# illini-robomaster/irmv_detection

Hardware: NVIDIA B200
Metric: frames/s (640^2 YOLOv8n+NMS+PnP) (higher is better)
Workload: dtype f16

## Files before the change

### irmv_detection_b200/csrc/common.cuh

```cuda
#pragma once
#include <cuda_fp16.h>
#include <cuda_runtime.h>
#include <stdint.h>

#include <string>
#include <vector>

namespace irmv {

constexpr int kNet = 640;
constexpr int kInC = 8;
constexpr int kRegMax = 16;
constexpr int kNumAnchors = 8400;
constexpr int kClsPad = 16;
constexpr int kMaxCand = 4096;

__host__ __device__ inline int pr_wp(int W) { return W + 1; }
__host__ __device__ inline long long pr_pixels(int B, int H, int W) { return ((long long)B * (H + 1) + 1) * (W + 1); }
__host__ __device__ inline long long pr_index(int b, int y, int x, int H, int W) {
  return ((long long)b * (H + 1) + 1 + y) * (W + 1) + x;
}
constexpr int kGuardFront = 384;
constexpr int kGuardBack = 1024;

void set_error(const std::string &msg);
bool cuda_ok(cudaError_t e, const char *what, const char *file, int line);

#define IRMV_CUDA(call)                                              \
  do {                                                               \
    if (!::irmv::cuda_ok((call), #call, __FILE__, __LINE__)) return 1; \
  } while (0)

struct PreprocessParams {
  const uint8_t *src;
  const uint8_t *const *src_indirect;
  __half *dst;
  uint8_t *rotated;
  int n, src_w, src_h;
  int frame0;
  int rev_order;
  int chan_order, rotate180, resize_mode, quantize_u8;
  int pad_x, pad_y, new_w, new_h;
};
inline void letterbox_geometry(int src_w, int src_h, int resize_mode, int *pad_x, int *pad_y, int *new_w, int *new_h) {
  *pad_x = *pad_y = 0; *new_w = *new_h = kNet;
  if (resize_mode != 1) return;
  const double rw = (double)kNet / src_w, rh = (double)kNet / src_h, r = rw < rh ? rw : rh;
  *new_w = (int)(src_w * r + 0.5); *new_h = (int)(src_h * r + 0.5);
  if (*new_w > kNet) *new_w = kNet;
  if (*new_h > kNet) *new_h = kNet;
  const double dw = (kNet - *new_w) / 2.0, dh = (kNet - *new_h) / 2.0;
  *pad_x = (int)(dw - 0.1 + 0.5); *pad_y = (int)(dh - 0.1 + 0.5);
  if (*pad_x < 0) *pad_x = 0;
  if (*pad_y < 0) *pad_y = 0;
}
cudaError_t launch_preprocess(const PreprocessParams &p, cudaStream_t s);
cudaError_t launch_rotate(const PreprocessParams &p, cudaStream_t s);
cudaError_t launch_stem(const PreprocessParams &p, const float *w, const float *bias, const uint32_t *fast_tab, __half *out,
                        long long out_pstride, __half *out2, long long out2_pstride, cudaStream_t s);
bool stem_bayer2x_applies(const PreprocessParams &p);
std::vector<uint32_t> stem_bayer2x_tables(const float *w, const float *bias, int src_h, int chan_order, int rotate180);
cudaError_t launch_stem_bayer2x(const PreprocessParams &p, int frame0, const uint32_t *tab, __half *out,
                                long long out_ps, __half *out2, long long out2_ps, cudaStream_t s);

struct ConvSeg {
  const __half *ptr;
  long long pstride;
  int c;
  int up;
  int runs;
};
__host__ __device__ inline int run_plane(int i, int runs) {
  return runs == 0 ? i : (((i >> (runs - 1)) << runs) + (i & ((1 << (runs - 1)) - 1)));
}

struct ConvParams {
  ConvSeg seg[2];
  int nseg;
  int B, H, W;
  int OH, OW;
  int k, stride, pad;
  int cin;
  int cout;
  int npad;
  int K;
  int kpad;
  int act;
  const __half *w_plain;
  const __half *w_tiled;
  const __half *w_raster;
  const int32_t *ktab;
  const float *bias;
  __half *out;
  long long out_pstride;
  int out_runs;
  const __half *res;
  long long res_pstride;
  int res_up;
  const __half *tail_w;
  const float *tail_bias;
  int tail_npad, tail_cout, tail_act;
  __half *tail_out;
  long long tail_out_pstride;
  __half *tail_out2;
  long long tail_out2_pstride;
  ConvSeg tail_ext;
  int in_parity;
  __half *out2;
  long long out2_pstride;
  int rev_tiles;
  int sync_mode;
  long long *trace;
  int trace_cap;
  const __half *w_raster_split;
  int split_ways;
};
cudaError_t launch_conv_direct(const ConvParams &p, cudaStream_t s);
cudaError_t launch_conv_tc(const ConvParams &p, int num_sms, cudaStream_t s);
size_t conv_tc_smem_bytes(const ConvParams &p, int *stages, int *b_resident);
bool conv_raster_fits(const ConvParams &p);
bool conv_raster_plan_info(const ConvParams &p, int num_sms, int out[8]);
cudaError_t launch_conv_raster(const ConvParams &p, int num_sms, cudaStream_t s);

__host__ __device__ inline int32_t ktab_meta(int tap, int seg, int valid, int plane) {
  return tap | (seg << 4) | (valid << 5) | (plane << 8);
}

struct DwParams {
  const __half *in;
  long long in_ps;
  __half *out;
  long long out_ps;
  const __half *w;
  const float *bias;
  int planes, B, H, W;
  int stride;
  int rev;
};
cudaError_t launch_dwconv3x3(const DwParams &p, cudaStream_t s);

struct ShuffleBlobLayout { int w1, w2, wa, dw, dwa, bias, bytes; };
__host__ __device__ inline ShuffleBlobLayout shuffle_blob_layout(int down, int cin, int h) {
  ShuffleBlobLayout L;
  L.w1 = 0;
  L.w2 = L.w1 + h * (cin + 8) * 2;
  L.wa = L.w2 + h * (h + 8) * 2;
  L.dw = L.wa + (down ? h * (cin + 8) * 2 : 0);
  L.dwa = L.dw + (h / 8) * 80 * 4;
  L.bias = L.dwa + (down ? (cin / 8) * 80 * 4 : 0);
  L.bytes = L.bias + (4 * h + cin) * 4;
  return L;
}
struct ShuffleUnitParams {
  int down;
  const __half *in;
  long long in_ps;
  __half *out;
  long long out_ps;
  int B, H, W;
  int cin, h;
  int first_plane, runs;
  const uint8_t *blob;
  int TH;
  int rev;
  int num_sms;
};
size_t shuffle_unit_smem(const ShuffleUnitParams &p);
int shuffle_unit_ctas_per_sm(const ShuffleUnitParams &p);
cudaError_t launch_shuffle_unit(const ShuffleUnitParams &p, cudaStream_t s);

cudaError_t launch_sppf_pool(__half *buf, int B, int H, int W, long long pstride, int c, cudaStream_t s);

struct HeadPtrs {
  const __half *box[3];
  const __half *cls[3];
  long long box_ps[3], cls_ps[3];
  int padded;
};
struct DetOut {
  int32_t *num_dets;
  float *boxes;
  float *scores;
  int32_t *classes;
  int32_t *index;
};
struct NmsScratch {
  float *boxes;
  unsigned long long *keys;
  int32_t *counts;
};
cudaError_t launch_decode(const HeadPtrs &h, int B, int nc, float score_thr, NmsScratch sc,
                          float *scores_or_null, cudaStream_t s);
cudaError_t launch_score_filter(const float *scores, int B, int A, int nc, float score_thr,
                                NmsScratch sc, cudaStream_t s);
cudaError_t launch_nms(NmsScratch sc, int B, int A, int nc, float iou_thr, int max_det, DetOut out,
                       cudaStream_t s);

struct ArmorOut {
  float pts[8];
  float center[2];
  float score;
  int32_t class_id;
  int32_t size;
  int32_t valid;
};
struct ArmorParams {
  const uint8_t *src;
  const uint8_t *const *src_indirect;
  int n, src_w, src_h, chan_order, rotate180;
  const int32_t *num;
  const float *boxes;
  const float *scores;
  const int32_t *classes;
  int max_det;
  float box_sx, box_sy, box_px, box_py;
  int binary_threshold;
  float min_ratio, max_ratio, max_angle;
  double min_small, max_small, min_large, max_large;
  ArmorOut *out;
  int *slot_locks;
  uint32_t *scratch;
  size_t scratch_words_per_cta;
  int grid;
  unsigned long long *prof;
};
int armors_grid(int num_sms);
size_t armors_scratch_words_per_cta(int src_w, int src_h);
size_t armors_scratch_total_words(int src_w, int src_h, int grid);
cudaError_t launch_extract_armors(const ArmorParams &p, cudaStream_t s);
cudaError_t launch_quads_from_armors(const ArmorOut *armors, int total, float sx, float sy, float *pts, float *centers, cudaStream_t s);
cudaError_t launch_mask_pose_ok(const ArmorOut *armors, int total, uint8_t *ok, cudaStream_t s);

struct PnpConsts {
  double fx, fy, cx, cy;
  double k1, k2, p1, p2, k3;
  double half_w[2], half_h[2];
};
struct PnpOut {
  double *rvec, *tvec;
  uint8_t *ok;
  double *quat;
  double *rvec2, *tvec2, *rmse;
  float *dist;
  const float *centers;
};
cudaError_t launch_pnp(const PnpConsts &c, const float *pts, int n, int large, PnpOut out,
                       cudaStream_t s);
cudaError_t launch_pnp_refine_lm(const PnpConsts &c, const float *pts, int n, int large, int max_iters, double *rvec,
                                 double *tvec, double *quat, cudaStream_t s);

}
```

### irmv_detection_b200/csrc/conv_raster.cu

```cuda
#include <cstdlib>

#include "common.cuh"

namespace irmv {
namespace {

constexpr int MAX_STAGES = 4;
constexpr int MAX_BSTAGES = 4;
constexpr int SMEM_BUDGET = 226 * 1024;

struct Bars {
  uint64_t full[MAX_STAGES];
  uint64_t empty[MAX_STAGES];
  uint64_t bw_full[MAX_BSTAGES];
  uint64_t bw_empty[MAX_BSTAGES];
  uint64_t tmem_full[2];
  uint64_t tmem_empty[2];
  uint64_t mid_full, mid_empty;
  uint64_t ext_full[2], ext_empty[2];
  uint64_t tail_full[2], tail_empty[2];
  uint64_t bfull;
  uint32_t tmem_base;
  uint32_t pad;
};

__device__ __forceinline__ uint32_t smem_u32(const void *p) { return (uint32_t)__cvta_generic_to_shared(p); }
__device__ __forceinline__ void mbar_init(uint64_t *bar, uint32_t count) {
  asm volatile("mbarrier.init.shared::cta.b64 [%0], %1;" ::"r"(smem_u32(bar)), "r"(count));
}
__device__ __forceinline__ void mbar_wait(uint64_t *bar, uint32_t parity) {
  asm volatile(
      "{\n"
      ".reg .pred P1;\n"
      "LAB_WAIT:\n"
      "mbarrier.try_wait.parity.shared::cta.b64 P1, [%0], %1, %2;\n"
      "@P1 bra DONE;\n"
      "bra LAB_WAIT;\n"
      "DONE:\n"
      "}" ::"r"(smem_u32(bar)), "r"(parity), "r"(0x989680u) : "memory");
}
__device__ __forceinline__ bool mbar_test(uint64_t *bar, uint32_t parity) {
  uint32_t ok;
  asm volatile(
      "{\n"
      ".reg .pred P1;\n"
      "mbarrier.test_wait.parity.shared::cta.b64 P1, [%1], %2;\n"
      "selp.u32 %0, 1, 0, P1;\n"
      "}" : "=r"(ok) : "r"(smem_u32(bar)), "r"(parity) : "memory");
  return ok != 0;
}
__device__ __forceinline__ void mbar_wait_warp(uint64_t *bar, uint32_t parity, int lane) {
  if (lane == 0) mbar_wait(bar, parity);
  __syncwarp();
}
__device__ __forceinline__ uint32_t elect_one() {
  uint32_t pred = 0;
  asm volatile(
      "{\n"
      ".reg .b32 %%rx;\n"
      ".reg .pred %%px;\n"
      "elect.sync %%rx|%%px, %1;\n"
      "@%%px mov.s32 %0, 1;\n"
      "}" : "+r"(pred) : "r"(0xffffffffu));
  return pred;
}
__device__ __forceinline__ void mbar_arrive(uint64_t *bar) {
  asm volatile("mbarrier.arrive.shared::cta.b64 _, [%0];" ::"r"(smem_u32(bar)) : "memory");
}
__device__ __forceinline__ void mbar_expect_tx(uint32_t bar, uint32_t bytes) {
  asm volatile("mbarrier.arrive.expect_tx.shared::cta.b64 _, [%0], %1;" ::"r"(bar), "r"(bytes) : "memory");
}
__device__ __forceinline__ void bulk_g2s(uint32_t dst, const void *src, uint32_t bytes, uint32_t bar) {
  asm volatile("cp.async.bulk.shared::cluster.global.mbarrier::complete_tx::bytes [%0], [%1], %2, [%3];"
               ::"r"(dst), "l"(src), "r"(bytes), "r"(bar) : "memory");
}
__device__ __forceinline__ void tc_fence_before() { asm volatile("tcgen05.fence::before_thread_sync;" ::: "memory"); }
__device__ __forceinline__ void tc_fence_after() { asm volatile("tcgen05.fence::after_thread_sync;" ::: "memory"); }
__device__ __forceinline__ void tc_commit(uint64_t *bar) {
  asm volatile("tcgen05.commit.cta_group::1.mbarrier::arrive::one.shared::cluster.b64 [%0];" ::"r"(smem_u32(bar)) : "memory");
}
__device__ __forceinline__ void tc_mma_f16(uint32_t tmem_d, uint32_t alo, uint32_t ahi, uint32_t blo, uint32_t bhi,
                                           uint32_t idesc, uint32_t accumulate) {
  asm volatile(
      "{\n"
      ".reg .pred p;\n"
      ".reg .b64 da, db;\n"
      "setp.ne.b32 p, %6, 0;\n"
      "mov.b64 da, {%1, %2};\n"
      "mov.b64 db, {%3, %4};\n"
      "tcgen05.mma.cta_group::1.kind::f16 [%0], da, db, %5, p;\n"
      "}" ::"r"(tmem_d), "r"(alo), "r"(ahi), "r"(blo), "r"(bhi), "r"(idesc), "r"(accumulate) : "memory");
}
__device__ __forceinline__ void tc_ld16(uint32_t taddr, uint32_t (&r)[16]) {
  asm volatile(
      "tcgen05.ld.sync.aligned.32x32b.x16.b32 "
      "{%0, %1, %2, %3, %4, %5, %6, %7, %8, %9, %10, %11, %12, %13, %14, %15}, [%16];"
      : "=r"(r[0]), "=r"(r[1]), "=r"(r[2]), "=r"(r[3]), "=r"(r[4]), "=r"(r[5]), "=r"(r[6]), "=r"(r[7]),
        "=r"(r[8]), "=r"(r[9]), "=r"(r[10]), "=r"(r[11]), "=r"(r[12]), "=r"(r[13]), "=r"(r[14]), "=r"(r[15])
      : "r"(taddr));
}
__device__ __forceinline__ void tc_ld_wait() { asm volatile("tcgen05.wait::ld.sync.aligned;" ::: "memory"); }

__device__ __forceinline__ uint32_t desc_lo(uint32_t saddr, uint32_t lbo_bytes) {
  return ((saddr & 0x3FFFFu) >> 4) | (((lbo_bytes >> 4) & 0x3FFFu) << 16);
}
constexpr uint32_t kDescHi = (128u >> 4) | (1u << 14);

struct RArgs {
  ConvParams p;
  int R, TM, PP, halo_front, npix_need;
  int NCH, NP, taps, Wp, Hp1;
  int q_begin, q_end, num_tiles, stages, tmem_cols, ctas_per_sm;
  int b_stream, b_stages;
  int nchunks, chunk_pairs;
  long long npix;
  uint32_t idesc, mul_wp, mul_hp1;
  uint32_t a_stage_bytes, b_bytes, b_tap_bytes, off_b, off_bias, off_bars;
  uint32_t tap_a[9];
  uint32_t off_mid, off_ext, off_bt, off_tbias, bt_bytes, tail_idesc;
  int ext_planes;
  int ext_stages;
  int rev;
  int tmem_tail0;
  int nsplit;
};

__device__ __forceinline__ void st_shared_v4(uint32_t addr, const uint4 &v) {
  asm volatile("st.shared.v4.b32 [%0], {%1, %2, %3, %4};" ::"r"(addr), "r"(v.x), "r"(v.y), "r"(v.z), "r"(v.w) : "memory");
}
__device__ __forceinline__ void st_shared_zero2(uint32_t addr, uint32_t plane_bytes) {
  const uint4 z = make_uint4(0, 0, 0, 0);
  st_shared_v4(addr, z);
  st_shared_v4(addr + plane_bytes, z);
}

template <bool ACT, int RES, bool MID = false>
__device__ __forceinline__ void epi_chunk(const uint32_t (&v32)[16], const float *hb, __half *o, long long out_ps,
                                          __half *o2, long long out2_ps, const uint4 &r0, const uint4 &r1,
                                          uint32_t mid = 0, uint32_t mid_plane_bytes = 0) {
  float b[16];
#pragma unroll
  for (int j = 0; j < 4; ++j) {
    const float4 t = *reinterpret_cast<const float4 *>(hb + 4 * j);
    b[4 * j] = t.x; b[4 * j + 1] = t.y; b[4 * j + 2] = t.z; b[4 * j + 3] = t.w;
  }
  if (RES == 2) {
    const float sc = ACT ? 0.5f : 1.0f;
    const __half2 *h0 = reinterpret_cast<const __half2 *>(&r0);
    const __half2 *h1 = reinterpret_cast<const __half2 *>(&r1);
#pragma unroll
    for (int t = 0; t < 4; ++t) {
      const float2 f0 = __half22float2(h0[t]), f1 = __half22float2(h1[t]);
      b[2 * t] = fmaf(f0.x, sc, b[2 * t]); b[2 * t + 1] = fmaf(f0.y, sc, b[2 * t + 1]);
      b[8 + 2 * t] = fmaf(f1.x, sc, b[8 + 2 * t]); b[8 + 2 * t + 1] = fmaf(f1.y, sc, b[8 + 2 * t + 1]);
    }
  }
  float v[16];
  if (ACT) {
#pragma unroll
    for (int j = 0; j < 16; ++j) {
      const float h = fmaf(__uint_as_float(v32[j]), 0.5f, b[j]);
      float t;
      asm("tanh.approx.f32 %0, %1;" : "=f"(t) : "f"(h));
      v[j] = fmaf(h, t, h);
    }
  } else {
#pragma unroll
    for (int j = 0; j < 16; ++j) v[j] = __uint_as_float(v32[j]) + b[j];
  }
  if (RES == 1) {
    const __half2 *h0 = reinterpret_cast<const __half2 *>(&r0);
    const __half2 *h1 = reinterpret_cast<const __half2 *>(&r1);
#pragma unroll
    for (int t = 0; t < 4; ++t) {
      const float2 f0 = __half22float2(h0[t]), f1 = __half22float2(h1[t]);
      v[2 * t] += f0.x; v[2 * t + 1] += f0.y;
      v[8 + 2 * t] += f1.x; v[8 + 2 * t + 1] += f1.y;
    }
  }
  __half2 hv[8];
#pragma unroll
  for (int t = 0; t < 8; ++t) hv[t] = __floats2half2_rn(v[2 * t], v[2 * t + 1]);
  if (o) {
    *reinterpret_cast<uint4 *>(o) = *reinterpret_cast<uint4 *>(&hv[0]);
    *reinterpret_cast<uint4 *>(o + out_ps) = *reinterpret_cast<uint4 *>(&hv[4]);
  }
  if (o2) {
    *reinterpret_cast<uint4 *>(o2) = *reinterpret_cast<uint4 *>(&hv[0]);
    *reinterpret_cast<uint4 *>(o2 + out2_ps) = *reinterpret_cast<uint4 *>(&hv[4]);
  }
  if (MID) {
    st_shared_v4(mid, *reinterpret_cast<uint4 *>(&hv[0]));
    st_shared_v4(mid + mid_plane_bytes, *reinterpret_cast<uint4 *>(&hv[4]));
  }
}

template <int R, int NEPI, bool ACT, int RES, int TAIL>
__global__ void __launch_bounds__((NEPI + 2) * 32, NEPI == 8 ? 2 : 1) conv_raster_kernel(const __grid_constant__ RArgs a) {
  constexpr int NTHREADS = (NEPI + 2) * 32;
  constexpr int TMA_WARP = NEPI, MMA_WARP = NEPI + 1;
  extern __shared__ __align__(1024) uint8_t smem[];
  const ConvParams &p = a.p;
  uint8_t *sA = smem;
  uint8_t *sB = smem + a.off_b;
  float *s_hb = reinterpret_cast<float *>(smem + a.off_bias);
  uint8_t *sMid = smem + a.off_mid;
  uint8_t *sExt = smem + a.off_ext;
  uint8_t *sBt = smem + a.off_bt;
  float *s_tb = reinterpret_cast<float *>(smem + a.off_tbias);
  Bars *bars = reinterpret_cast<Bars *>(smem + a.off_bars);
  const int tid = threadIdx.x, warp = tid >> 5, lane = tid & 31;
  const int npad = p.npad;
  const int nsplit = a.nsplit;
  const int bid = nsplit > 1 ? (int)(blockIdx.x / (unsigned)nsplit) : (int)blockIdx.x;
  const int gsz = nsplit > 1 ? (int)(gridDim.x / (unsigned)nsplit) : (int)gridDim.x;
  const int split = nsplit > 1 ? (int)(blockIdx.x % (unsigned)nsplit) : 0;
  const float *const bias_g = p.bias + split * npad;
  const uint8_t *const w_g = reinterpret_cast<const uint8_t *>(p.w_raster) + (size_t)split * a.b_bytes;
  long long *trow = (p.trace && tid == 0 && (blockIdx.x == 0 || blockIdx.x == gridDim.x - 1))
                        ? p.trace + (size_t)(p.trace_cap + (blockIdx.x == 0 ? 15 : 14)) * 8 : nullptr;
  if (trow) {
    trow[0] = clock64();
    unsigned long long g;
    asm volatile("mov.u64 %0, %%globaltimer;" : "=l"(g));
    trow[3] = (long long)g;
  }

  asm volatile("griddepcontrol.launch_dependents;" ::: "memory");
  for (int i = tid; i < npad; i += NTHREADS) s_hb[i] = ACT ? 0.5f * bias_g[i] : bias_g[i];
  if (TAIL)
    for (int i = tid; i < p.tail_npad; i += NTHREADS) s_tb[i] = TAIL == 2 ? 0.5f * p.tail_bias[i] : p.tail_bias[i];
  if (tid == 0) {
    for (int s = 0; s < a.stages; ++s) {
      mbar_init(&bars->full[s], 1);
      mbar_init(&bars->empty[s], 1);
    }
    for (int s = 0; s < MAX_BSTAGES; ++s) {
      mbar_init(&bars->bw_full[s], 1);
      mbar_init(&bars->bw_empty[s], 1);
    }
    for (int i = 0; i < 2; ++i) {
      mbar_init(&bars->tmem_full[i], 1);
      mbar_init(&bars->tmem_empty[i], NEPI);
    }
    mbar_init(&bars->bfull, 1);
    mbar_init(&bars->mid_full, NEPI);
    mbar_init(&bars->mid_empty, 1);
    for (int i = 0; i < 2; ++i) {
      mbar_init(&bars->ext_full[i], 1);
      mbar_init(&bars->ext_empty[i], 1);
    }
    for (int i = 0; i < 2; ++i) {
      mbar_init(&bars->tail_full[i], 1);
      mbar_init(&bars->tail_empty[i], NEPI);
    }
    asm volatile("fence.mbarrier_init.release.cluster;" ::: "memory");
  }
  if (warp == MMA_WARP) {
    asm volatile("tcgen05.alloc.cta_group::1.sync.aligned.shared::cta.b32 [%0], %1;"
                 ::"r"(smem_u32(&bars->tmem_base)), "r"((uint32_t)a.tmem_cols) : "memory");
    asm volatile("tcgen05.relinquish_alloc_permit.cta_group::1.sync.aligned;" ::: "memory");
  }
  tc_fence_before();
  __syncthreads();
  tc_fence_after();
  const uint32_t tmem_base = bars->tmem_base;
  if (trow) trow[1] = clock64();
  if (warp == TMA_WARP && !a.b_stream && elect_one()) {
    const uint32_t bar = smem_u32(&bars->bfull), sB_u = smem_u32(sB);
    mbar_expect_tx(bar, a.b_bytes + (TAIL ? a.bt_bytes : 0u));
    for (uint32_t off = 0; off < a.b_bytes; off += 65536u) {
      const uint32_t n = a.b_bytes - off < 65536u ? a.b_bytes - off : 65536u;
      bulk_g2s(sB_u + off, w_g + off, n, bar);
    }
    if (TAIL) bulk_g2s(smem_u32(sBt), p.tail_w, a.bt_bytes, bar);
  }
  asm volatile("griddepcontrol.wait;" ::: "memory");

  if (warp < NEPI) {
    constexpr int NSUB = NEPI / 4;
    const int ew = warp & 3, sub = warp >> 2;
    const int chunk_shift = 31 - __clz(npad >> 4);
    const int chunk_mask = (npad >> 4) - 1;
    const int items = R << chunk_shift;
    const uint32_t lane_base = tmem_base + ((uint32_t)(ew * 32) << 16);
    __half *const out = p.out ? p.out + (long long)(split * (npad >> 3)) * p.out_pstride : nullptr;
    const __half *const res = p.res ? p.res + (long long)(split * (npad >> 3)) * p.res_pstride : nullptr;
    const long long out_ps = p.out_pstride, res_ps = p.res_pstride;
    const int orl = p.out_runs;
    const long long out_ps_pair = orl == 1 ? 2 * out_ps : out_ps;
    const int cout = p.cout;
    const int Wp = a.Wp, Hp1 = a.Hp1, W = p.OW, q_end = a.q_end, TM = a.TM;
    __half *const out2 = p.out2;
    const long long out2_ps = p.out2_pstride;
    const int Wp2 = (p.OW >> 1) + 1, Hp2 = (p.OH >> 1) + 1, cpl = cout >> 3;
    const uint32_t mul_wp = a.mul_wp, mul_hp1 = a.mul_hp1;
    const int q_lane = a.q_begin + ew * 32 + lane;
    const int num_tiles = a.num_tiles;
    long long *const trace = p.trace;
    const int trace_cap = p.trace_cap;
    auto valid_mask = [&](int q_tile) -> uint32_t {
      uint32_t m = 0;
#pragma unroll
      for (int r = 0; r < R; ++r) {
        const int qi = q_tile + r * 128;
        const uint32_t row = (uint32_t)(((uint64_t)(uint32_t)qi * mul_wp) >> 34);
        const int x = qi - (int)row * Wp;
        const uint32_t img = (uint32_t)(((uint64_t)row * mul_hp1) >> 34);
        const int yrow = (int)row - (int)img * Hp1;
        if (qi < q_end && x < W && yrow != 0) m |= 1u << r;
      }
      return m;
    };
    const int tnp = TAIL ? p.tail_npad : 16;
    const int tshift = 31 - __clz(tnp >> 4), tmask = (tnp >> 4) - 1;
    __half *const tout = p.tail_out;
    const long long tout_ps = p.tail_out_pstride;
    __half *const tout2 = p.tail_out2;
    const long long tout2_ps = p.tail_out2_pstride;
    const int tcout = p.tail_cout;
    auto tail_epilogue = [&](int jt, int tile_j) {
      const int tb = jt & 1;
      const int q_tile = q_lane + tile_j * TM;
      const uint32_t okm = valid_mask(q_tile);
      mbar_wait_warp(&bars->tail_full[tb], (uint32_t)(jt >> 1) & 1u, lane);
      tc_fence_after();
      const uint32_t tcol = lane_base + (uint32_t)(a.tmem_tail0 + tb * R * tnp);
      const int items2 = R << tshift;
      const uint4 z = make_uint4(0, 0, 0, 0);
      for (int w = sub; w < items2; w += NSUB) {
        const int r = w >> tshift, c0 = (w & tmask) << 4;
        uint32_t v[16];
        tc_ld16(tcol + (uint32_t)(r * tnp + c0), v);
        tc_ld_wait();
        if (((okm >> r) & 1u) && c0 < tcout) {
          __half *o = tout ? tout + (long long)(c0 >> 3) * tout_ps + (long long)(q_tile + r * 128) * 8 : nullptr;
          __half *o2 = nullptr;
          if (tout2) {
            const int qi = q_tile + r * 128;
            const uint32_t row = (uint32_t)(((uint64_t)(uint32_t)qi * mul_wp) >> 34);
            const int x = qi - (int)row * Wp;
            const uint32_t img = (uint32_t)(((uint64_t)row * mul_hp1) >> 34);
            const int y = (int)row - (int)img * Hp1 - 1;
            const int px2 = ((int)img * Hp2 + 1 + (y >> 1)) * Wp2 + (x >> 1);
            o2 = tout2 + (long long)(((y & 1) * 2 + (x & 1)) * (tcout >> 3) + (c0 >> 3)) * tout2_ps + (long long)px2 * 8;
          }
          epi_chunk<TAIL == 2, false>(v, s_tb + c0, o, tout_ps, o2, tout2_ps, z, z);
        }
      }
      tc_fence_before();
      __syncwarp();
      if (lane == 0) mbar_arrive(&bars->tail_empty[tb]);
    };
    int it = 0, prev_tile = -1;
    for (int tseq = bid; tseq < num_tiles; tseq += gsz, ++it) {
      const int tile = a.rev ? num_tiles - 1 - tseq : tseq;
      const int buf = it & 1;
      const uint32_t aph = (uint32_t)(it >> 1) & 1u;
      const bool tr = trace && blockIdx.x == 0 && tid == 0 && it < trace_cap;
      const int q_tile = q_lane + tile * TM;
      const uint32_t okmask = valid_mask(q_tile);
      __half *const out_q = out + (long long)q_tile * 8;
      const __half *const res_q = RES == 1 ? res + (long long)q_tile * 8 : nullptr;
      mbar_wait_warp(&bars->tmem_full[buf], aph, lane);
      if (TAIL) mbar_wait_warp(&bars->mid_empty, (uint32_t)(it & 1) ^ 1u, lane);
      tc_fence_after();
      if (tr) trace[it * 8 + 6] = clock64();
      const uint32_t tcol0 = lane_base + (uint32_t)(buf * R * npad);
      const uint32_t mid_lane = smem_u32(sMid) + (uint32_t)(ew * 32 + lane) * 16u;
      struct Item { int c0; bool ok; __half *o, *o2; uint32_t mid; uint4 r0, r1; };
      auto setup = [&](int w, Item &t) -> uint32_t {
        const int r = w >> chunk_shift;
        t.c0 = (w & chunk_mask) << 4;
        t.ok = ((okmask >> r) & 1u) && t.c0 < cout;
        const long long off = (long long)run_plane(t.c0 >> 3, orl) * out_ps + r * 1024;
        t.o = out ? out_q + off : nullptr;
        t.o2 = nullptr;
        t.mid = TAIL ? mid_lane + (uint32_t)((t.c0 >> 3) * TM + r * 128) * 16u : 0u;
        if (out2) {
          const int qi = q_tile + r * 128;
          const uint32_t row = (uint32_t)(((uint64_t)(uint32_t)qi * mul_wp) >> 34);
          const int x = qi - (int)row * Wp;
          const uint32_t img = (uint32_t)(((uint64_t)row * mul_hp1) >> 34);
          const int y = (int)row - (int)img * Hp1 - 1;
          const int px2 = ((int)img * Hp2 + 1 + (y >> 1)) * Wp2 + (x >> 1);
          t.o2 = out2 + (long long)(((y & 1) * 2 + (x & 1)) * cpl + (t.c0 >> 3)) * out2_ps + (long long)px2 * 8;
        }
        if (RES == 1 && t.ok) {
          const __half *rp = res_q + (long long)(t.c0 >> 3) * res_ps + r * 1024;
          t.r0 = *reinterpret_cast<const uint4 *>(rp);
          t.r1 = *reinterpret_cast<const uint4 *>(rp + res_ps);
        }
        if (RES == 2 && t.ok) {
          const int qi = q_tile + r * 128;
          const uint32_t row = (uint32_t)(((uint64_t)(uint32_t)qi * mul_wp) >> 34);
          const int x = qi - (int)row * Wp;
          const uint32_t img = (uint32_t)(((uint64_t)row * mul_hp1) >> 34);
          const int y = (int)row - (int)img * Hp1 - 1;
          const int px2 = ((int)img * Hp2 + 1 + (y >> 1)) * Wp2 + (x >> 1);
          const __half *rp = res + (long long)(t.c0 >> 3) * res_ps + (long long)px2 * 8;
          t.r0 = __ldg(reinterpret_cast<const uint4 *>(rp));
          t.r1 = __ldg(reinterpret_cast<const uint4 *>(rp + res_ps));
        }
        return tcol0 + (uint32_t)(r * npad + t.c0);
      };
      uint32_t va[16], vb[16];
      Item ia, ib;
      ia.r0 = ia.r1 = ib.r0 = ib.r1 = make_uint4(0, 0, 0, 0);
      int w = sub;
      if (w < items) tc_ld16(setup(w, ia), va);
      while (w < items) {
        tc_ld_wait();
        const bool more_b = w + NSUB < items;
        if (more_b) tc_ld16(setup(w + NSUB, ib), vb);
        if (ia.ok) epi_chunk<ACT, RES, TAIL != 0>(va, s_hb + ia.c0, ia.o, out_ps_pair, ia.o2, out2_ps, ia.r0, ia.r1, ia.mid, (uint32_t)TM * 16u);
        else if (TAIL) st_shared_zero2(ia.mid, (uint32_t)TM * 16u);
        if (!more_b) break;
        tc_ld_wait();
        const bool more_a = w + 2 * NSUB < items;
        if (more_a) tc_ld16(setup(w + 2 * NSUB, ia), va);
        if (ib.ok) epi_chunk<ACT, RES, TAIL != 0>(vb, s_hb + ib.c0, ib.o, out_ps_pair, ib.o2, out2_ps, ib.r0, ib.r1, ib.mid, (uint32_t)TM * 16u);
        else if (TAIL) st_shared_zero2(ib.mid, (uint32_t)TM * 16u);
        if (!more_a) break;
        w += 2 * NSUB;
      }
      if (TAIL) asm volatile("fence.proxy.async.shared::cta;" ::: "memory");
      tc_fence_before();
      __syncwarp();
      if (lane == 0) {
        mbar_arrive(&bars->tmem_empty[buf]);
        if (TAIL) mbar_arrive(&bars->mid_full);
      }
      if (tr) trace[it * 8 + 7] = clock64();
      if (TAIL && it > 0) tail_epilogue(it - 1, prev_tile);
      prev_tile = tile;
    }
    if (TAIL && it > 0) tail_epilogue(it - 1, prev_tile);
  } else if (warp == TMA_WARP) {
    if (elect_one()) {
      const uint32_t sA_u = smem_u32(sA), sB_u = smem_u32(sB);
      int s = 0, itl = 0, bs = 0;
      uint32_t ph = 0, bph = 0;
      const uint32_t plane_bytes = (uint32_t)a.npix_need * 16u;
      const uint32_t pitch_bytes = (uint32_t)a.PP * 16u;
      const uint32_t tile_tx = plane_bytes * (uint32_t)a.NP;
      const int n0 = p.in_parity ? a.NP : p.seg[0].c >> 3, n1 = p.nseg > 1 ? p.seg[1].c >> 3 : 0;
      const size_t ps0 = (size_t)p.seg[0].pstride * 2, ps1 = (size_t)p.seg[1].pstride * 2;
      const int rl0 = p.in_parity ? 0 : p.seg[0].runs;
      const uint32_t ext_bytes = (uint32_t)a.TM * 16u;
      const uint32_t ext_buf_bytes = ext_bytes * (uint32_t)a.ext_planes;
      auto issue_ext = [&](int j, int tile_j) {
        const int eb = a.ext_stages == 2 ? (j & 1) : 0;
        const uint32_t bar = smem_u32(&bars->ext_full[eb]);
        mbar_expect_tx(bar, ext_buf_bytes);
        uint32_t dst = smem_u32(sExt) + (uint32_t)eb * ext_buf_bytes;
        const uint8_t *src = reinterpret_cast<const uint8_t *>(p.tail_ext.ptr) + ((long long)a.q_begin + (long long)tile_j * a.TM) * 16;
        const size_t pse = (size_t)p.tail_ext.pstride * 2;
        for (int c = 0; c < a.ext_planes; ++c, dst += ext_bytes, src += pse) bulk_g2s(dst, src, ext_bytes, bar);
      };
      auto issue_main = [&](int tile, int itl) {
        const bool tr = p.trace && blockIdx.x == 0 && itl < p.trace_cap;
        const long long qlo = (long long)a.q_begin + (long long)tile * a.TM - a.halo_front;
        if (tr) p.trace[itl * 8 + 1] = clock64();
        const uint32_t bar = smem_u32(&bars->full[s]);
        mbar_expect_tx(bar, tile_tx);
        uint32_t dst = sA_u + (uint32_t)s * a.a_stage_bytes;
        const uint8_t *src = reinterpret_cast<const uint8_t *>(p.seg[0].ptr) + qlo * 16;
        if (rl0 == 0) {
          for (int c = 0; c < n0; ++c, dst += pitch_bytes, src += ps0) bulk_g2s(dst, src, plane_bytes, bar);
        } else {
          for (int c = 0; c < n0; ++c, dst += pitch_bytes) bulk_g2s(dst, src + (size_t)run_plane(c, rl0) * ps0, plane_bytes, bar);
        }
        src = reinterpret_cast<const uint8_t *>(p.seg[1].ptr) + qlo * 16;
        for (int c = 0; c < n1; ++c, dst += pitch_bytes, src += ps1) bulk_g2s(dst, src, plane_bytes, bar);
        if (tr) p.trace[itl * 8 + 2] = clock64();
        if (++s == a.stages) { s = 0; ph ^= 1u; }
      };
      auto tile_of = [&](int seq) { return a.rev ? a.num_tiles - 1 - seq : seq; };
      if (TAIL && a.ext_planes) {
        const int mine = a.num_tiles > bid ? (a.num_tiles - 1 - bid) / gsz + 1 : 0;
        int mi = 0, ei = 0;
        while (mi < mine || ei < mine) {
          bool progressed = false;
          if (mi < mine && mbar_test(&bars->empty[s], ph ^ 1u)) {
            if (p.trace && blockIdx.x == 0 && mi < p.trace_cap) p.trace[mi * 8 + 0] = clock64();
            issue_main(tile_of(bid + mi * gsz), mi);
            ++mi;
            progressed = true;
          }
          if (ei < mine) {
            const int eb = a.ext_stages == 2 ? (ei & 1) : 0;
            const uint32_t eph = a.ext_stages == 2 ? ((uint32_t)(ei >> 1) & 1u) : ((uint32_t)ei & 1u);
            if (mbar_test(&bars->ext_empty[eb], eph ^ 1u)) {
              issue_ext(ei, tile_of(bid + ei * gsz));
              ++ei;
              progressed = true;
            }
          }
          if (!progressed) __nanosleep(64);
        }
      } else {
        for (int tseq = bid; tseq < a.num_tiles; tseq += gsz, ++itl) {
          const int tile = tile_of(tseq);
          if (p.trace && blockIdx.x == 0 && itl < p.trace_cap) p.trace[itl * 8 + 0] = clock64();
          mbar_wait(&bars->empty[s], ph ^ 1u);
          issue_main(tile, itl);
          if (a.b_stream) {
            const uint8_t *wsrc = w_g;
            for (int t = 0; t < a.nchunks; ++t, wsrc += a.b_tap_bytes) {
              mbar_wait(&bars->bw_empty[bs], bph ^ 1u);
              const uint32_t bbar = smem_u32(&bars->bw_full[bs]);
              mbar_expect_tx(bbar, a.b_tap_bytes);
              bulk_g2s(sB_u + (uint32_t)bs * a.b_tap_bytes, wsrc, a.b_tap_bytes, bbar);
              if (++bs == a.b_stages) { bs = 0; bph ^= 1u; }
            }
          }
        }
      }
    }
  } else {
    if (!a.b_stream) mbar_wait_warp(&bars->bfull, 0, lane);
    int it = 0, s = 0, bs = 0;
    uint32_t ph = 0, bph = 0;
    const uint32_t a_lo0 = desc_lo(smem_u32(sA), (uint32_t)a.PP * 16u);
    const uint32_t b_lo0 = desc_lo(smem_u32(sB), (uint32_t)npad * 16u);
    const uint32_t a_stage_u = a.a_stage_bytes >> 4;
    const uint32_t a_pair_u = 2u * (uint32_t)a.PP;
    const uint32_t b_pair_u = 2u * (uint32_t)npad;
    const uint32_t b_tap_u = a.b_tap_bytes >> 4;
    const int pairs = a.chunk_pairs, nchunks = a.nchunks;
    const int tnp = TAIL ? p.tail_npad : 16;
    const uint32_t mid_lo0 = desc_lo(smem_u32(sMid), (uint32_t)a.TM * 16u);
    const uint32_t ext_lo0 = desc_lo(smem_u32(sExt), (uint32_t)a.TM * 16u);
    const uint32_t bt_lo0 = desc_lo(smem_u32(sBt), (uint32_t)tnp * 16u);
    auto issue_tail = [&](int j) {
      const int tb = j & 1;
      const int eb = a.ext_stages == 2 ? (j & 1) : 0;
      const uint32_t eph = a.ext_stages == 2 ? ((uint32_t)(j >> 1) & 1u) : ((uint32_t)j & 1u);
      mbar_wait_warp(&bars->mid_full, (uint32_t)j & 1u, lane);
      if (a.ext_planes) mbar_wait_warp(&bars->ext_full[eb], eph, lane);
      mbar_wait_warp(&bars->tail_empty[tb], ((uint32_t)(j >> 1) & 1u) ^ 1u, lane);
      tc_fence_after();
      if (elect_one()) {
        const uint32_t td0 = tmem_base + (uint32_t)(a.tmem_tail0 + tb * R * tnp);
        uint32_t bl = bt_lo0, acc = 0;
        uint32_t al = ext_lo0 + (uint32_t)eb * (uint32_t)(a.ext_planes * a.TM);
        for (int kk = 0; kk < (a.ext_planes >> 1); ++kk, al += 2u * (uint32_t)a.TM, bl += 2u * (uint32_t)tnp) {
#pragma unroll
          for (int r = 0; r < R; ++r)
            tc_mma_f16(td0 + (uint32_t)(r * tnp), al + (uint32_t)(r * 128), kDescHi, bl, kDescHi, a.tail_idesc, acc);
          acc = 1;
        }
        al = mid_lo0;
        for (int kk = 0; kk < (npad >> 4); ++kk, al += 2u * (uint32_t)a.TM, bl += 2u * (uint32_t)tnp) {
#pragma unroll
          for (int r = 0; r < R; ++r)
            tc_mma_f16(td0 + (uint32_t)(r * tnp), al + (uint32_t)(r * 128), kDescHi, bl, kDescHi, a.tail_idesc, acc);
          acc = 1;
        }
        tc_commit(&bars->tail_full[tb]);
        tc_commit(&bars->mid_empty);
        if (a.ext_planes) tc_commit(&bars->ext_empty[eb]);
      }
      __syncwarp();
    };
    for (int tile = bid; tile < a.num_tiles; tile += gsz, ++it) {
      const int buf = it & 1;
      const uint32_t aph = (uint32_t)(it >> 1) & 1u;
      const bool tr = p.trace && blockIdx.x == 0 && lane == 0 && it < p.trace_cap;
      if (tr) p.trace[it * 8 + 3] = clock64();
      mbar_wait_warp(&bars->tmem_empty[buf], aph ^ 1u, lane);
      mbar_wait_warp(&bars->full[s], ph, lane);
      tc_fence_after();
      if (tr) p.trace[it * 8 + 4] = clock64();
      const uint32_t tmem_d0 = tmem_base + (uint32_t)(buf * R * npad);
      const uint32_t a_stage_lo = a_lo0 + (uint32_t)s * a_stage_u;
      if (!a.b_stream) {
        if (elect_one()) {
          uint32_t acc = 0;
          uint32_t bl_t = b_lo0;
          for (int t = 0; t < nchunks; ++t, bl_t += b_tap_u) {
            uint32_t al = a_stage_lo + a.tap_a[t], bl = bl_t;
            for (int j = 0; j < pairs; ++j, al += a_pair_u, bl += b_pair_u) {
#pragma unroll
              for (int r = 0; r < R; ++r)
                tc_mma_f16(tmem_d0 + (uint32_t)(r * npad), al + (uint32_t)(r * 128), kDescHi, bl, kDescHi, a.idesc, acc);
              acc = 1;
            }
          }
          tc_commit(&bars->empty[s]);
          tc_commit(&bars->tmem_full[buf]);
        }
        __syncwarp();
      } else {
        for (int t = 0; t < nchunks; ++t) {
          mbar_wait_warp(&bars->bw_full[bs], bph, lane);
          tc_fence_after();
          if (elect_one()) {
            uint32_t al = a_stage_lo + a.tap_a[t], bl = b_lo0 + (uint32_t)bs * b_tap_u;
            for (int j = 0; j < pairs; ++j, al += a_pair_u, bl += b_pair_u) {
#pragma unroll
              for (int r = 0; r < R; ++r)
                tc_mma_f16(tmem_d0 + (uint32_t)(r * npad), al + (uint32_t)(r * 128), kDescHi, bl, kDescHi, a.idesc,
                           (t | j) != 0 ? 1u : 0u);
            }
            tc_commit(&bars->bw_empty[bs]);
            if (t == nchunks - 1) {
              tc_commit(&bars->empty[s]);
              tc_commit(&bars->tmem_full[buf]);
            }
          }
          __syncwarp();
          if (++bs == a.b_stages) { bs = 0; bph ^= 1u; }
        }
      }
      if (tr) p.trace[it * 8 + 5] = clock64();
      if (++s == a.stages) { s = 0; ph ^= 1u; }
      if (TAIL && it > 0) issue_tail(it - 1);
    }
    if (TAIL && it > 0) issue_tail(it - 1);
  }

  tc_fence_before();
  __syncthreads();
  if (trow) {
    trow[2] = clock64();
    unsigned long long g;
    asm volatile("mov.u64 %0, %%globaltimer;" : "=l"(g));
    trow[4] = (long long)g;
  }
  if (warp == MMA_WARP) {
    asm volatile("tcgen05.dealloc.cta_group::1.sync.aligned.b32 %0, %1;" ::"r"(tmem_base), "r"((uint32_t)a.tmem_cols) : "memory");
  }
}

bool plan(const ConvParams &p_in, int num_sms, RArgs &a) {
  ConvParams p = p_in;
  a.nsplit = 1;
  static const bool split_env = !getenv("IRMV_NO_NSPLIT");
  if (split_env && p.w_raster_split && p.split_ways > 1 && p.stride == 1 && !p.in_parity && !p.tail_w && !p.out2 && !p.out_runs &&
      !p.seg[0].runs && !p.res_up && p.out && p.cout == p.npad && p.npad % (16 * p.split_ways) == 0) {
    const long long m = (long long)p.B * (p.OH + 1) * (p.OW + 1) - (p.OW + 1);
    if ((m + 127) / 128 * p.split_ways <= num_sms) {
      a.nsplit = p.split_ways;
      p.w_raster = p.w_raster_split;
      p.cout /= a.nsplit;
      p.npad /= a.nsplit;
    }
  }
  const bool s2 = p.stride == 2;
  if (s2) {
    if (!p.in_parity || p.k != 3 || p.pad != 1 || p.nseg != 1 || (p.H & 1) || (p.W & 1)) return false;
  } else {
    if (p.in_parity || p.stride != 1 || !(p.k == 1 || p.k == 3) || (p.k == 3 && p.pad != 1) || (p.k == 1 && p.pad != 0)) return false;
  }
  if (p.cin % 16 != 0 || p.npad % 16 != 0 || p.npad > 256) return false;
  for (int i = 0; i < p.nseg; ++i) if (p.seg[i].up || p.seg[i].c % 8) return false;
  if (p.OW + 2 + 8 > kGuardFront || p.cout % 16 != 0) return false;
  if (p.out2 && ((p.OH & 1) || (p.OW & 1))) return false;
  if (p.res_up && (!p.res || !p.act || p.tail_w || s2 || (p.OH & 1) || (p.OW & 1))) return false;
  if ((p.out_runs || p.seg[0].runs) && (p.out2 || p.res || p.tail_w || p.in_parity || p.nseg != 1)) return false;
  a.p = p;
  a.rev = p.rev_tiles;
  a.NCH = p.cin / 8;
  a.NP = s2 ? 4 * a.NCH : a.NCH;
  a.taps = p.k * p.k;
  a.Wp = p.OW + 1;
  a.Hp1 = p.OH + 1;
  a.npix = pr_pixels(p.B, p.OH, p.OW);
  a.q_begin = a.Wp;
  a.q_end = (p.B * (p.OH + 1)) * a.Wp;
  const long long Mr = (long long)a.q_end - a.q_begin;
  a.b_bytes = (uint32_t)((size_t)a.taps * p.cin * p.npad * 2);
  a.nchunks = a.taps;
  a.chunk_pairs = a.NCH >> 1;
  a.b_tap_bytes = (uint32_t)((size_t)p.cin * p.npad * 2);
  const bool tail = p.tail_w != nullptr;
  if (tail && (p.tail_npad % 16 || p.tail_npad > 256 || p.tail_cout % 16 || p.cout != p.npad || (!p.tail_out && !p.tail_out2))) return false;
  if (tail && p.res && !(p.act && p.tail_act)) return false;
  const int tnp = tail ? p.tail_npad : 0;
  const int ext_c = tail ? p.tail_ext.c : 0;
  if (ext_c % 16 || (tail && p.tail_ext.up) || (tail && p.tail_out2 && ((p.OH & 1) || (p.OW & 1)))) return false;
  a.ext_planes = ext_c / 8;
  a.bt_bytes = tail ? (uint32_t)((size_t)(p.npad + ext_c) * tnp * 2) : 0u;
  int ext_stages = 1;
  auto tail_bytes = [&](int R) { return tail ? (size_t)a.bt_bytes + (size_t)(p.npad + ext_c * ext_stages) * 128 * R * 2 + 256 : (size_t)0; };
  const size_t misc = (size_t)p.npad * 4 + (size_t)tnp * 4 + sizeof(Bars) + 1024 + 256;
  const int halo = p.k == 3 ? (s2 ? a.Wp + 1 : 2 * a.Wp + 2) : 0;
  const int halo_front = p.k == 3 ? a.Wp + 1 : 0;
  const int delta = (((a.q_begin - halo_front) % 8) + 8) % 8;
  auto plane_pixels = [&](int R) { return (128 * R + halo + delta + 7) & ~7; };
  auto stage_bytes = [&](int R) { return (size_t)a.NP * plane_pixels(R) * 16; };
  int best_R = 0;
  a.b_stream = 0;
  static const int rmax_env = getenv("IRMV_RMAX") ? atoi(getenv("IRMV_RMAX")) : 4;
  static const bool ext2_env = !getenv("IRMV_EXT1");
  for (int R = 4; R >= 1 && !best_R; R >>= 1) {
    if (R > rmax_env) continue;
    if (2 * R * (p.npad + tnp) > 512) continue;
    long long tiles = (Mr + 128 * R - 1) / (128 * R);
    if (R > 1 && tiles < 2LL * num_sms) continue;
    for (ext_stages = (ext_c && ext2_env) ? 2 : 1; ext_stages >= 1; --ext_stages) {
      if (a.b_bytes + tail_bytes(R) + 2 * stage_bytes(R) + misc > (size_t)SMEM_BUDGET) continue;
      best_R = R;
      break;
    }
  }
  if (ext_stages < 1) ext_stages = 1;
  a.ext_stages = ext_stages;
  if (!best_R && tail) return false;
  if (!best_R && !getenv("IRMV_NO_BSTREAM")) {
    if (p.k == 1) {
      if (a.NCH % 8 != 0 || a.NCH / 8 > 9) return false;
      a.nchunks = a.NCH / 8;
      a.chunk_pairs = 4;
      a.b_tap_bytes = (uint32_t)((size_t)64 * p.npad * 2);
    }
    for (int R = 4; R >= 1; R >>= 1) {
      if (2 * R * p.npad > 512) continue;
      if (2 * (size_t)a.b_tap_bytes + stage_bytes(R) + misc > (size_t)SMEM_BUDGET) continue;
      long long tiles = (Mr + 128 * R - 1) / (128 * R);
      if (R > 1 && tiles < (long long)num_sms) continue;
      best_R = R;
      a.b_stream = 1;
      break;
    }
  }
  if (!best_R) return false;
  a.R = best_R;
  a.TM = 128 * a.R;
  a.halo_front = halo_front + delta;
  a.npix_need = plane_pixels(a.R);
  a.PP = a.npix_need;
  a.a_stage_bytes = (uint32_t)stage_bytes(a.R);
  int cols = 2 * a.R * (p.npad + tnp), alloc = 32;
  while (alloc < cols) alloc <<= 1;
  a.tmem_cols = alloc;
  a.tmem_tail0 = 2 * a.R * p.npad;
  a.num_tiles = (int)((Mr + a.TM - 1) / a.TM);
  size_t b_smem = a.b_bytes;
  if (a.b_stream) {
    a.ctas_per_sm = 1;
    size_t left = (size_t)SMEM_BUDGET - misc;
    a.stages = (left >= 2 * (size_t)a.a_stage_bytes + 2 * (size_t)a.b_tap_bytes) ? 2 : 1;
    left -= (size_t)a.stages * a.a_stage_bytes;
    a.b_stages = (int)(left / a.b_tap_bytes);
    if (a.b_stages > MAX_BSTAGES) a.b_stages = MAX_BSTAGES;
    b_smem = (size_t)a.b_stages * a.b_tap_bytes;
  } else {
    const size_t half_budget = 112 * 1024;
    const size_t fixed = a.b_bytes + tail_bytes(a.R) + misc;
    const bool two = !getenv("IRMV_ONE_CTA") && alloc <= 256 && fixed + 2 * (size_t)a.a_stage_bytes <= half_budget;
    a.ctas_per_sm = two ? 2 : 1;
    const size_t budget = two ? half_budget : (size_t)SMEM_BUDGET;
    a.stages = (int)((budget - fixed) / a.a_stage_bytes);
    if (a.stages > MAX_STAGES) a.stages = MAX_STAGES;
    a.b_stages = 0;
  }
  a.idesc = (1u << 4) | ((uint32_t)(p.npad >> 3) << 17) | ((uint32_t)(128 >> 4) << 24);
  a.mul_wp = (uint32_t)(((1ull << 34) + (uint64_t)a.Wp - 1) / (uint64_t)a.Wp);
  a.mul_hp1 = (uint32_t)(((1ull << 34) + (uint64_t)a.Hp1 - 1) / (uint64_t)a.Hp1);
  a.off_b = (uint32_t)((size_t)a.stages * a.a_stage_bytes);
  a.off_mid = (uint32_t)((a.off_b + b_smem + 127u) & ~(size_t)127u);
  a.off_ext = a.off_mid + (tail ? (uint32_t)((size_t)p.npad * a.TM * 2) : 0u);
  a.off_bt = a.off_ext + (uint32_t)((size_t)ext_c * a.ext_stages * a.TM * 2);
  a.off_bias = (uint32_t)((a.off_bt + a.bt_bytes + 127u) & ~(size_t)127u);
  a.off_tbias = a.off_bias + (uint32_t)p.npad * 4;
  a.off_bars = (a.off_tbias + (uint32_t)tnp * 4 + 15u) & ~15u;
  a.tail_idesc = (1u << 4) | ((uint32_t)((tail ? tnp : 16) >> 3) << 17) | ((uint32_t)(128 >> 4) << 24);
  for (int t = 0; t < 9; ++t) {
    const int ky = t / 3, kx = t % 3;
    if (s2) {
      const int g = (ky != 1) * 2 + (kx != 1);
      a.tap_a[t] = (uint32_t)(g * a.NCH * a.PP + delta + (ky == 0 ? 0 : a.Wp) + (kx == 0 ? 0 : 1));
    } else if (a.taps == 9) {
      a.tap_a[t] = (uint32_t)(delta + ky * a.Wp + kx);
    } else {
      a.tap_a[t] = (uint32_t)(delta + t * 8 * a.PP);
    }
  }
  return true;
}

template <int R, int NEPI, bool ACT, int RES, int TAIL>
cudaError_t launch_k(const RArgs &a, int grid, size_t smem, cudaStream_t s) {
  {
    cudaError_t e = cudaFuncSetAttribute(conv_raster_kernel<R, NEPI, ACT, RES, TAIL>, cudaFuncAttributeMaxDynamicSharedMemorySize, 227 * 1024);
    if (e != cudaSuccess) return e;
  }
  static const bool pdl = !getenv("IRMV_NO_PDL");
  cudaLaunchConfig_t cfg{};
  cfg.gridDim = dim3((unsigned)grid);
  cfg.blockDim = dim3((NEPI + 2) * 32);
  cfg.dynamicSmemBytes = smem;
  cfg.stream = s;
  cudaLaunchAttribute attr[1];
  attr[0].id = cudaLaunchAttributeProgrammaticStreamSerialization;
  attr[0].val.programmaticStreamSerializationAllowed = 1;
  cfg.attrs = attr;
  cfg.numAttrs = pdl ? 1 : 0;
  return cudaLaunchKernelEx(&cfg, conv_raster_kernel<R, NEPI, ACT, RES, TAIL>, a);
}

template <int R, int NEPI>
cudaError_t launch_r(const RArgs &a, int grid, size_t smem, cudaStream_t s) {
  const bool act = a.p.act != 0, res = a.p.res != nullptr;
  if (res && a.p.res_up) {
    if (!act || a.p.tail_w) return cudaErrorInvalidValue;
    return launch_k<R, NEPI, true, 2, 0>(a, grid, smem, s);
  }
  if (a.p.tail_w) {
    if (res) {
      if (!act || !a.p.tail_act) return cudaErrorInvalidValue;
      return launch_k<R, NEPI, true, 1, 2>(a, grid, smem, s);
    }
    if (a.p.tail_act) return act ? launch_k<R, NEPI, true, 0, 2>(a, grid, smem, s) : launch_k<R, NEPI, false, 0, 2>(a, grid, smem, s);
    return act ? launch_k<R, NEPI, true, 0, 1>(a, grid, smem, s) : launch_k<R, NEPI, false, 0, 1>(a, grid, smem, s);
  }
  if (act) return res ? launch_k<R, NEPI, true, 1, 0>(a, grid, smem, s) : launch_k<R, NEPI, true, 0, 0>(a, grid, smem, s);
  return res ? launch_k<R, NEPI, false, 1, 0>(a, grid, smem, s) : launch_k<R, NEPI, false, 0, 0>(a, grid, smem, s);
}

}

bool conv_raster_plan_info(const ConvParams &p, int num_sms, int out[8]) {
  RArgs a;
  if (!p.w_raster || !plan(p, num_sms, a)) return false;
  out[0] = a.R; out[1] = a.ctas_per_sm == 2 ? 8 : 16; out[2] = a.b_stream; out[3] = a.ctas_per_sm; out[4] = a.stages;
  out[5] = a.b_stages; out[6] = p.tail_w ? (p.tail_act ? 2 : 1) : 0; out[7] = a.num_tiles;
  return true;
}

bool conv_raster_fits(const ConvParams &p) {
  RArgs a;
  return p.w_raster != nullptr && plan(p, 148, a);
}

cudaError_t launch_conv_raster(const ConvParams &p, int num_sms, cudaStream_t s) {
  RArgs a;
  if (!plan(p, num_sms, a)) return cudaErrorInvalidValue;
  const size_t smem = (size_t)a.off_bars + sizeof(Bars) + 64;
  const int slots = num_sms * a.ctas_per_sm / a.nsplit;
  const int grid = (a.num_tiles < slots ? a.num_tiles : slots) * a.nsplit;
  if (a.ctas_per_sm == 2) {
    switch (a.R) {
      case 4: return launch_r<4, 8>(a, grid, smem, s);
      case 2: return launch_r<2, 8>(a, grid, smem, s);
      default: return launch_r<1, 8>(a, grid, smem, s);
    }
  }
  switch (a.R) {
    case 4: return launch_r<4, 16>(a, grid, smem, s);
    case 2: return launch_r<2, 16>(a, grid, smem, s);
    default: return launch_r<1, 16>(a, grid, smem, s);
  }
}

}
```

### irmv_detection_b200/csrc/engine.cu

```cuda
#include <algorithm>
#include <atomic>
#include <cstdio>
#include <cstdlib>
#include <cstring>
#include <chrono>
#include <exception>
#include <map>
#include <memory>
#include <mutex>
#include <string>
#include <vector>

#include "../../include/irmv_cabi.h"
#include "common.cuh"

namespace irmv {

static thread_local std::string g_err;
void set_error(const std::string &msg) { g_err = msg; }
bool cuda_ok(cudaError_t e, const char *what, const char *file, int line) {
  if (e == cudaSuccess) return true;
  char buf[512];
  snprintf(buf, sizeof buf, "%s:%d: %s -> %s", file, line, what, cudaGetErrorString(e));
  set_error(buf);
// ... 154 lines not shown
               i, c.cin, c.cout, c.k, c.stride, c.act, w.cin, w.cout, w.k, w.stride, w.act);
      set_error(buf);
      return false;
    }
  }
  return true;
}

HostConv make_conv(const std::vector<const FileConv *> &parts, int cin_pad,
                   const std::vector<int> &seg_c) {
  HostConv h;
  const FileConv &f0 = *parts[0];
  h.cin_eff = cin_pad; h.k = f0.k; h.stride = f0.stride; h.act = f0.act;
  int cout_real = 0;
  for (auto *p : parts) cout_real += p->cout;
  h.cout = (cout_real + 7) / 8 * 8;
  h.npad = (cout_real + 15) / 16 * 16;
  if (h.cout < h.npad) h.cout = h.npad;
  h.K = h.k * h.k * cin_pad;
  h.kpad = (h.K + 63) / 64 * 64;
  h.seg_c = seg_c;
  h.w_plain.assign((size_t)h.npad * h.kpad, __float2half(0.f));
  h.bias.assign(h.npad, 0.f);
  int n0 = 0;
  for (auto *p : parts) {
    for (int n = 0; n < p->cout; ++n) {
      h.bias[n0 + n] = p->b[n];
      for (int c = 0; c < p->cin; ++c)
        for (int ky = 0; ky < p->k; ++ky)
          for (int kx = 0; kx < p->k; ++kx) {
            float v = p->w[(((size_t)n * p->cin + c) * p->k + ky) * p->k + kx];
            size_t kk = (size_t)(ky * p->k + kx) * cin_pad + c;
            h.w_plain[(size_t)(n0 + n) * h.kpad + kk] = __float2half(v);
          }
    }
    n0 += p->cout;
  }
  const int KB = h.kpad / 64;
  h.w_tiled.assign((size_t)KB * h.npad * 64, __float2half(0.f));
  for (int kb = 0; kb < KB; ++kb)
    for (int n = 0; n < h.npad; ++n)
      for (int kk = 0; kk < 64; ++kk) {
        int chunk = (kk >> 3) ^ (n & 7);
        h.w_tiled[((size_t)kb * h.npad + n) * 64 + chunk * 8 + (kk & 7)] =
            h.w_plain[(size_t)n * h.kpad + kb * 64 + kk];
      }
  {
    const int taps = h.k * h.k, nch = cin_pad / 8;
    h.w_raster.assign((size_t)taps * nch * h.npad * 8, __float2half(0.f));
    for (int t = 0; t < taps; ++t)
      for (int c = 0; c < nch; ++c)
        for (int n = 0; n < h.npad; ++n)
          for (int e = 0; e < 8; ++e)
            h.w_raster[(((size_t)t * nch + c) * h.npad + n) * 8 + e] =
                h.w_plain[(size_t)n * h.kpad + (size_t)t * cin_pad + c * 8 + e];
  }
  h.ktab.assign((size_t)(h.kpad / 8) * 3, -1);
  for (int q = 0; q < h.K / 8; ++q) {
    int kk = q * 8, tap = kk / cin_pad, c = kk % cin_pad;
    int sg = 0, off = c;
    if (seg_c.size() > 1 && c >= seg_c[0]) { sg = 1; off = c - seg_c[0]; }
    h.ktab[q * 3 + 0] = tap; h.ktab[q * 3 + 1] = sg; h.ktab[q * 3 + 2] = off;
  }
  return h;
}

FileConv slice_cin(const FileConv &f, int c0, int c1, bool keep_bias_act) {
  FileConv r = f;
  const int kk = f.k * f.k;
  r.cin = c1 - c0;
  r.w.assign((size_t)f.cout * r.cin * kk, 0.f);
  for (int n = 0; n < f.cout; ++n)
    for (int c = c0; c < c1; ++c)
      for (int t = 0; t < kk; ++t) r.w[((size_t)n * r.cin + (c - c0)) * kk + t] = f.w[((size_t)n * f.cin + c) * kk + t];
  if (!keep_bias_act) { r.act = 0; std::fill(r.b.begin(), r.b.end(), 0.f); }
  return r;
}

FileConv permuted(const FileConv &f, const std::vector<int> &in_map, const std::vector<int> &out_map) {
  FileConv r = f;
  const int kk = f.k * f.k;
  for (int n = 0; n < f.cout; ++n) {
    const int ln = out_map.empty() ? n : out_map[n];
    r.b[n] = f.b[ln];
    for (int c = 0; c < f.cin; ++c) {
      const int lc = in_map.empty() ? c : in_map[c];
      for (int t = 0; t < kk; ++t) r.w[((size_t)n * f.cin + c) * kk + t] = f.w[((size_t)ln * f.cin + lc) * kk + t];
    }
  }
  return r;
}

struct HostDw {
  int c = 0, stride = 1;
  std::vector<__half> w;
  std::vector<float> b;
  __half *d_w = nullptr;
  float *d_b = nullptr;
};

HostDw make_dw(const FileConv &f, const std::vector<int> &map) {
  HostDw h;
  h.c = f.cout; h.stride = f.stride;
  h.w.assign((size_t)f.cout * 9, __float2half(0.f));
  h.b.assign(f.cout, 0.f);
  for (int pc = 0; pc < f.cout; ++pc) {
    const int lc = map.empty() ? pc : map[pc];
    h.b[pc] = f.b[lc];
    for (int t = 0; t < 9; ++t) h.w[((size_t)(pc / 8) * 9 + t) * 8 + pc % 8] = __float2half(f.w[(size_t)lc * 9 + t]);
  }
  return h;
}

bool upload(HostConv &h) {
  auto up = [](void **d, const void *src, size_t bytes) {
    if (!cuda_ok(dev_malloc(d, bytes), "dev_malloc(weights)", __FILE__, __LINE__)) return false;
    return cuda_ok(cudaMemcpy(*d, src, bytes, cudaMemcpyHostToDevice), "cudaMemcpy(weights)",
                   __FILE__, __LINE__);
  };
  if (h.npad >= 128 && h.npad % 64 == 0 && !h.w_raster.empty() && h.w_raster.size() % ((size_t)h.npad * 8) == 0) {
    const int ways = 4, ns = h.npad / ways;
    const size_t rows = h.w_raster.size() / ((size_t)h.npad * 8);
    std::vector<__half> sp(h.w_raster.size());
    for (int sl = 0; sl < ways; ++sl)
      for (size_t r = 0; r < rows; ++r)
        for (int n = 0; n < ns; ++n)
          for (int j = 0; j < 8; ++j)
            sp[(((size_t)sl * rows + r) * ns + n) * 8 + j] = h.w_raster[(r * h.npad + (size_t)sl * ns + n) * 8 + j];
    if (!up((void **)&h.d_raster_split, sp.data(), sp.size() * 2)) return false;
    h.split_ways = ways;
  }
  return up((void **)&h.d_plain, h.w_plain.data(), h.w_plain.size() * 2) &&
         up((void **)&h.d_tiled, h.w_tiled.data(), h.w_tiled.size() * 2) &&
         up((void **)&h.d_raster, h.w_raster.data(), h.w_raster.size() * 2) &&
         up((void **)&h.d_bias, h.bias.data(), h.bias.size() * 4);
}

struct Tensor {
  __half *p = nullptr;
  long long pstride = 0;
  int H = 0, W = 0, C = 0;
  __half *pp = nullptr;
  long long pp_stride = 0;
  bool parity_only = false;
  std::vector<int> cmap;
};

struct Op {
  enum Kind { CONV, POOL, DW, SHUF } kind = CONV;
  DwParams dw{};
  ShuffleUnitParams su{};
  ConvParams cp{};
  bool raster = false;
  int stream = 0, wait = -1, signal = -1;
  __half *pool_buf = nullptr;
  int pH = 0, pW = 0, pC = 0;
  long long pStride = 0;
};

struct DetPack {
  size_t bytes = 0;
  uint8_t *dev = nullptr;
  int S = 0, max_det = 0;
  int32_t *num() const { return reinterpret_cast<int32_t *>(dev); }
  float *boxes() const { return reinterpret_cast<float *>(dev + off_boxes()); }
  float *scores() const { return reinterpret_cast<float *>(dev + off_scores()); }
  int32_t *classes() const { return reinterpret_cast<int32_t *>(dev + off_classes()); }
  int32_t *index() const { return reinterpret_cast<int32_t *>(dev + off_index()); }
  size_t off_boxes() const { return ((size_t)S * 4 + 15) & ~(size_t)15; }
  size_t off_scores() const { return off_boxes() + (size_t)S * max_det * 16; }
  size_t off_classes() const { return off_scores() + (size_t)S * max_det * 4; }
  size_t off_index() const { return off_classes() + (size_t)S * max_det * 4; }
  void init(int s, int md) { S = s; max_det = md; bytes = off_index() + (size_t)S * max_det * 4; }
};

struct Lane {
  cudaStream_t stream = nullptr;
  cudaEvent_t done = nullptr;
  std::vector<void *> allocs;
  struct Raster { const __half *p; long long pstride; int planes, H, W; };
  std::vector<Raster> rasters;
  std::map<std::string, Tensor> taps;
  std::vector<Op> ops;
  Tensor in8, stem_out;
  HeadPtrs heads{};
  NmsScratch nms{};
  DetPack det;
  const uint8_t **src_word = nullptr;
  uint8_t *rotated = nullptr;
  std::map<int, cudaGraphExec_t> graphs;
  static constexpr int kSide = 9, kSig = 6;
  cudaStream_t side[kSide] = {};
  cudaEvent_t side_done[kSide] = {}, sig[kSig] = {};
  int launches_per_replay = 0;
  float *pnp_pts = nullptr;
  double *pnp_rvec = nullptr, *pnp_tvec = nullptr;
  uint8_t *pnp_ok = nullptr;
  double *pnp_quat = nullptr;
  float *pnp_dist = nullptr;
  float *pnp_centers = nullptr;
  const __half *kpt[3] = {nullptr, nullptr, nullptr};
  float *kpts = nullptr;
  ArmorOut *armors = nullptr;
  uint32_t *armor_scratch = nullptr;
  cudaEvent_t stage_ev[6] = {nullptr, nullptr, nullptr, nullptr, nullptr, nullptr};
};

__global__ void set_src_kernel(const uint8_t **word, const uint8_t *ptr) { *word = ptr; }

__global__ void __launch_bounds__(256) check_padding_kernel(const __half *p, long long pstride, int planes, int S, int H, int W,
                                                            unsigned long long *bad) {
  const long long real = pr_pixels(S, H, W), total = (long long)kGuardFront + real + kGuardBack;
  const int plane = blockIdx.y;
  const uint4 *base = reinterpret_cast<const uint4 *>(p + (long long)plane * pstride) - kGuardFront;
  unsigned long long n = 0;
  for (long long i = (long long)blockIdx.x * blockDim.x + threadIdx.x; i < total; i += (long long)gridDim.x * blockDim.x) {
    const long long q = i - kGuardFront;
    bool must_be_zero = q < 0 || q >= real;
    if (!must_be_zero) {
      const long long row = q / (W + 1);
      const int x = (int)(q - row * (W + 1));
      must_be_zero = x == W || row % (H + 1) == 0;
    }
    if (must_be_zero) {
      const uint4 v = base[i];
      n += (v.x | v.y | v.z | v.w) != 0u;
    }
  }
  if (n) atomicAdd(bad, n);
  (void)planes;
}

__global__ void quads_from_dets_kernel(const int32_t *num, const float *boxes, int n, int max_det,
                                       float sx, float sy, float px, float py, float *pts) {
  int i = blockIdx.x * blockDim.x + threadIdx.x;
  if (i >= n * max_det) return;
  int f = i / max_det, k = i - f * max_det;
  float4 b = make_float4(150.f + px, 140.f + py, 200.f + px, 160.f + py);
  if (k < num[f]) b = reinterpret_cast<const float4 *>(boxes)[i];
  float x1 = (b.x - px) * sx, y1 = (b.y - py) * sy, x2 = (b.z - px) * sx, y2 = (b.w - py) * sy;
  float4 *o = reinterpret_cast<float4 *>(pts + (size_t)i * 8);
  o[0] = make_float4(x1, y2, x1, y1);
  o[1] = make_float4(x2, y1, x2, y2);
}

__global__ void kpts_from_dets_kernel(const int32_t *num, const int32_t *index, int n, int max_det, int nc,
                                      const __half *k0, const __half *k1, const __half *k2, float *kpts) {
  const int i = blockIdx.x * blockDim.x + threadIdx.x;
  if (i >= n * max_det) return;
  const int f = i / max_det, k = i - f * max_det;
  float4 lo = make_float4(0.f, 0.f, 0.f, 0.f), hi = lo;
  if (k < num[f]) {
    int a = index[i] / nc;
    const __half *base = k0;
    int hw = 80;
    float stride = 8.f;
    if (a >= 8000) { a -= 8000; base = k2; hw = 20; stride = 32.f; }
    else if (a >= 6400) { a -= 6400; base = k1; hw = 40; stride = 16.f; }
    const int gy = a / hw, gx = a - gy * hw;
    const uint4 raw = *reinterpret_cast<const uint4 *>(base + pr_index(f, gy, gx, hw, hw) * 8);
    const __half2 *h = reinterpret_cast<const __half2 *>(&raw);
    float v[8];
#pragma unroll
    for (int j = 0; j < 4; ++j) {
      const float2 p = __half22float2(h[j]);
      v[2 * j] = __fmul_rn(__fadd_rn(__fmul_rn(p.x, 2.f), (float)gx), stride);
      v[2 * j + 1] = __fmul_rn(__fadd_rn(__fmul_rn(p.y, 2.f), (float)gy), stride);
    }
    lo = make_float4(v[0], v[1], v[2], v[3]);
    hi = make_float4(v[4], v[5], v[6], v[7]);
  }
  float4 *o = reinterpret_cast<float4 *>(kpts + (size_t)i * 8);
  o[0] = lo; o[1] = hi;
}

__global__ void quads_from_kpts_kernel(const int32_t *num, const float *kpts, int n, int max_det, float sx, float sy,
                                       float px, float py, float *pts) {
  const int i = blockIdx.x * blockDim.x + threadIdx.x;
  if (i >= n * max_det) return;
  const int f = i / max_det, k = i - f * max_det;
  float q[8] = {150.f, 160.f, 150.f, 140.f, 200.f, 140.f, 200.f, 160.f};
  if (k < num[f]) {
#pragma unroll
    for (int j = 0; j < 4; ++j) {
      q[2 * j] = (kpts[(size_t)i * 8 + 2 * j] - px) * sx;
      q[2 * j + 1] = (kpts[(size_t)i * 8 + 2 * j + 1] - py) * sy;
    }
  }
  float4 *o = reinterpret_cast<float4 *>(pts + (size_t)i * 8);
  o[0] = make_float4(q[0], q[1], q[2], q[3]);
  o[1] = make_float4(q[4], q[5], q[6], q[7]);
}

}
}

using namespace irmv;

constexpr int kSets = 3;

struct irmv_engine {
  irmv_engine_config cfg{};
  int nc = IRMV_NUM_CLASSES;
  int num_sms = 148;
  int S = 1, L = 1;
  size_t frame_bytes = 0;
// ... 19 lines not shown
    cudaEvent_t done = nullptr;
    std::vector<cudaEvent_t> h2d;
    int n = 0;
    long long ticket = -1;
    bool in_flight = false;
  } sets[kSets];
  cudaStream_t copy_stream = nullptr;
  long long next_ticket = 0;
  size_t res_bytes = 0;
  size_t res_frame_stride = 0;
  double profile_ms = 0.0, device_ms = 0.0;
  bool pnp_on = false;
  bool fused_stem = true;
  float *d_stem_w = nullptr, *d_stem_b = nullptr;
  uint32_t *d_stem_tab = nullptr;
  PnpConsts pnp_c{};
  float pnp_sx = 1.f, pnp_sy = 1.f, pnp_px = 0.f, pnp_py = 0.f;
  float corner_sx = 1.f, corner_sy = 1.f;
  bool pose = false;
  bool armors_on = false;
  irmv_armor_params armor_prm{};
  int last_slot = -1;
  int last_n = 0;
  bool rotated_on = false;
  uint8_t *rot_dev = nullptr;
  std::vector<uint8_t *> rot_host;
  std::vector<char> rot_valid;
  std::vector<irmv_bbox> parse_tmp;
  unsigned long long h2d_bytes = 0, d2h_bytes = 0;
};

namespace {

bool lane_alloc(Lane &ln, void **p, size_t bytes) {
  if (!cuda_ok(dev_malloc(p, bytes), "dev_malloc(activation)", __FILE__, __LINE__)) return false;
  ln.allocs.push_back(*p);
  return cuda_ok(cudaMemset(*p, 0, bytes), "cudaMemset", __FILE__, __LINE__);
}

bool new_tensor(Lane &ln, int S, int H, int W, int C, Tensor &t, const char *tap = nullptr) {
  t.H = H; t.W = W; t.C = C;
  const size_t plane_px = ((size_t)kGuardFront + (size_t)pr_pixels(S, H, W) + kGuardBack + 7) & ~(size_t)7;
  t.pstride = (long long)plane_px * 8;
  __half *base = nullptr;
  if (!lane_alloc(ln, (void **)&base, (size_t)(C / 8) * plane_px * 16)) return false;
  t.p = base + (size_t)kGuardFront * 8;
  ln.rasters.push_back({t.p, t.pstride, C / 8, H, W});
  if (tap) ln.taps[tap] = t;
  return true;
}

bool add_parity_twin(Lane &ln, int S, Tensor &t, bool only) {
  t.parity_only = only;
  const size_t plane_px = ((size_t)kGuardFront + (size_t)pr_pixels(S, t.H / 2, t.W / 2) + kGuardBack + 7) & ~(size_t)7;
  t.pp_stride = (long long)plane_px * 8;
  __half *base = nullptr;
  if (!lane_alloc(ln, (void **)&base, (size_t)(4 * (t.C / 8)) * plane_px * 16)) return false;
  t.pp = base + (size_t)kGuardFront * 8;
  ln.rasters.push_back({t.pp, t.pp_stride, 4 * (t.C / 8), t.H / 2, t.W / 2});
  return true;
}

struct SegRef { const Tensor *t; int coff; int c; int up; };

void add_conv(irmv_engine *e, Lane &ln, HostConv &hc, std::vector<SegRef> in, int H, int W,
              const Tensor &out, int out_coff, const Tensor *res = nullptr, int res_coff = 0, int res_up = 0) {
  Op op;
  op.kind = Op::CONV;
  ConvParams &p = op.cp;
  p.nseg = (int)in.size();
  int cin = 0;
  for (int i = 0; i < p.nseg; ++i) {
    p.seg[i].ptr = in[i].t->p + (long long)(in[i].coff / 8) * in[i].t->pstride;
    p.seg[i].pstride = in[i].t->pstride;
    p.seg[i].c = in[i].c; p.seg[i].up = in[i].up;
    cin += in[i].c;
  }
  if (p.nseg == 1) p.seg[1] = p.seg[0];
  p.B = e->S; p.H = H; p.W = W;
  p.k = hc.k; p.stride = hc.stride; p.pad = hc.k / 2;
  p.OH = (H + 2 * p.pad - hc.k) / hc.stride + 1;
  p.OW = (W + 2 * p.pad - hc.k) / hc.stride + 1;
  p.cin = cin; p.cout = hc.cout; p.npad = hc.npad; p.K = hc.K; p.kpad = hc.kpad; p.act = hc.act;
  p.w_plain = hc.d_plain; p.w_tiled = hc.d_tiled; p.w_raster = hc.d_raster; p.bias = hc.d_bias;
  p.w_raster_split = hc.d_raster_split; p.split_ways = hc.split_ways;
  {
    const int nq = hc.kpad / 8;
    std::vector<int32_t> tab((size_t)nq * 2, 0);
    for (int q = 0; q < nq; ++q) {
      int tap = hc.ktab[q * 3 + 0], sg = hc.ktab[q * 3 + 1], off = hc.ktab[q * 3 + 2];
      if (tap < 0) { tab[q * 2 + 0] = 0; tab[q * 2 + 1] = ktab_meta(0, 0, 0, 0); continue; }
      const ConvSeg &g = p.seg[sg];
      int ky = tap / hc.k, kx = tap % hc.k;
      tab[q * 2 + 0] = g.up ? 0 : (ky - p.pad) * (W + 1) + (kx - p.pad);
      tab[q * 2 + 1] = ktab_meta(tap, sg, 1, off / 8);
    }
    int32_t *d = nullptr;
    dev_malloc((void **)&d, tab.size() * 4);
    cudaMemcpy(d, tab.data(), tab.size() * 4, cudaMemcpyHostToDevice);
    ln.allocs.push_back(d);
    p.ktab = d;
  }
  p.out = out.p + (long long)(out_coff / 8) * out.pstride; p.out_pstride = out.pstride;
  p.res = res ? res->p + (long long)(res_coff / 8) * res->pstride : nullptr;
  p.res_pstride = res ? res->pstride : 0;
  p.res_up = res ? res_up : 0;
  p.sync_mode = 0;
  p.trace = nullptr; p.trace_cap = 0;
  p.in_parity = 0;
  p.out2 = nullptr; p.out2_pstride = 0;
  if (out.pp && out_coff == 0 && hc.cout == out.C) {
    p.out2 = out.pp; p.out2_pstride = out.pp_stride;
    if (out.parity_only) p.out = nullptr;
  }
  if (hc.stride == 2 && p.nseg == 1 && in[0].t->pp && in[0].coff == 0 && in[0].c == in[0].t->C &&
      !getenv("IRMV_NO_RASTER") && !getenv("IRMV_NO_S2_RASTER")) {
    ConvParams q = p;
    q.in_parity = 1;
    q.seg[0].ptr = in[0].t->pp; q.seg[0].pstride = in[0].t->pp_stride;
    q.seg[1] = q.seg[0];
    if (conv_raster_fits(q)) p = q;
    else if (in[0].t->parity_only) fprintf(stderr, "irmv: internal: stride-2 consumer of a parity-only tensor does not fit the raster kernel\n");
  }
  op.raster = conv_raster_fits(p) && !getenv("IRMV_NO_RASTER");
  if (p.out2 && !op.raster) { p.out2 = nullptr; p.out = out.p; }
  ln.ops.push_back(op);
}

bool add_c2f(irmv_engine *e, Lane &ln, size_t &ci, std::vector<SegRef> in, int H, int W, int c2,
             int n, bool shortcut, Tensor &out, const char *tap, int parity_out = 0) {
  const int c = c2 / 2;
  Tensor buf, tmp;
  if (!new_tensor(ln, e->S, H, W, (2 + n) * c, buf) || !new_tensor(ln, e->S, H, W, c, tmp) ||
      !new_tensor(ln, e->S, H, W, c2, out, tap))
    return false;
  if (parity_out) {
    if (!add_parity_twin(ln, e->S, out, parity_out == 1)) return false;
    if (tap) ln.taps[tap] = out;
  }
  HostConv &cv1 = *e->convs[ci++];
  bool split = false;
  if (cv1.up_a && in.size() == 2 && in[0].up && !in[1].up) {
    Tensor ya;
    if (!new_tensor(ln, e->S, H / 2, W / 2, cv1.cout, ya)) return false;
    add_conv(e, ln, *cv1.up_a, {{in[0].t, in[0].coff, in[0].c, 0}}, H / 2, W / 2, ya, 0);
    const bool ok_a = ln.ops.back().raster;
    add_conv(e, ln, *cv1.up_b, {in[1]}, H, W, buf, 0, &ya, 0, 1);
    if (ok_a && ln.ops.back().raster) split = true;
    else { ln.ops.pop_back(); ln.ops.pop_back(); }
  }
  if (!split) add_conv(e, ln, cv1, in, H, W, buf, 0);
  for (int i = 0; i < n; ++i) {
    add_conv(e, ln, *e->convs[ci++], {{&buf, (1 + i) * c, c, 0}}, H, W, tmp, 0);
    add_conv(e, ln, *e->convs[ci++], {{&tmp, 0, c, 0}}, H, W, buf, (2 + i) * c,
             shortcut ? &buf : nullptr, (1 + i) * c);
  }
  add_conv(e, ln, *e->convs[ci++], {{&buf, 0, (2 + n) * c, 0}}, H, W, out, 0);
  return true;
}

void fuse_tails(irmv_engine *e, Lane &ln) {
  if (e->cfg.conv_impl == IRMV_CONV_DIRECT || e->cfg.reserved[1] || getenv("IRMV_NO_TAIL")) return;
  auto overlaps = [](const __half *a0, const __half *a1, const __half *b0, const __half *b1) { return a0 < b1 && b0 < a1; };
  for (size_t i = 0; i + 1 < ln.ops.size(); ++i) {
    Op &m = ln.ops[i];
    const Op &t = ln.ops[i + 1];
    if (m.kind != Op::CONV || t.kind != Op::CONV || !m.raster || !t.raster) continue;
    const ConvParams &tp = t.cp;
    ConvParams mp = m.cp;
    if (tp.k != 1 || tp.stride != 1 || tp.nseg != 1 || tp.res || tp.in_parity || tp.seg[0].up || tp.tail_w) continue;
    if (mp.out2 || mp.tail_w || !mp.out) continue;
    if (tp.seg[0].runs || tp.out_runs || mp.seg[0].runs || mp.out_runs) continue;
    const int ext = tp.seg[0].c - mp.cout;
    if (ext < 0 || tp.seg[0].pstride != mp.out_pstride) continue;
    if (tp.seg[0].ptr + (long long)(ext / 8) * tp.seg[0].pstride != mp.out) continue;
    if (tp.H != mp.OH || tp.W != mp.OW) continue;
    const __half *o0 = mp.out, *o1 = mp.out + (long long)(mp.cout / 8) * mp.out_pstride;
    bool other = false;
    for (size_t j = 0; j < ln.ops.size() && !other; ++j) {
      if (j == i || j == i + 1) continue;
      const Op &q = ln.ops[j];
      if (q.kind == Op::POOL) { other = overlaps(o0, o1, q.pool_buf, q.pool_buf + 4LL * (q.pC / 8) * q.pStride); continue; }
      if (q.kind == Op::DW) { other = overlaps(o0, o1, q.dw.in, q.dw.in + (long long)q.dw.planes * q.dw.in_ps); continue; }
      if (q.kind == Op::SHUF) { other = overlaps(o0, o1, q.su.in, q.su.in + (long long)(q.su.down ? q.su.cin / 8 : q.su.h / 4) * q.su.in_ps); continue; }
      for (int sgi = 0; sgi < q.cp.nseg; ++sgi) {
        const ConvSeg &g = q.cp.seg[sgi];
        if (!q.cp.in_parity && overlaps(o0, o1, g.ptr, g.ptr + (long long)(g.c / 8) * g.pstride)) other = true;
      }
      if (q.cp.res && overlaps(o0, o1, q.cp.res, q.cp.res + (long long)(q.cp.cout / 8) * q.cp.res_pstride)) other = true;
    }
    for (int h = 0; h < 3 && !other; ++h)
      if (ln.heads.box[h] == mp.out || ln.heads.cls[h] == mp.out) other = true;
    if (other) continue;
    mp.tail_w = tp.w_raster; mp.tail_bias = tp.bias; mp.tail_npad = tp.npad; mp.tail_cout = tp.cout; mp.tail_act = tp.act;
    mp.tail_out = tp.out; mp.tail_out_pstride = tp.out_pstride;
    mp.tail_out2 = tp.out2; mp.tail_out2_pstride = tp.out2_pstride;
    mp.tail_ext = tp.seg[0]; mp.tail_ext.c = ext;
    mp.out = nullptr;
    if (!conv_raster_fits(mp)) continue;
    m.cp = mp;
    if (t.signal >= 0) m.signal = t.signal;
    for (auto it = ln.taps.begin(); it != ln.taps.end();)
      it = (it->second.p == o0) ? ln.taps.erase(it) : std::next(it);
    ln.ops.erase(ln.ops.begin() + (long)i + 1);
  }
}

bool build_lane(irmv_engine *e, Lane &ln) {
  const int S = e->S;
  if (!cuda_ok(cudaStreamCreateWithFlags(&ln.stream, cudaStreamNonBlocking), "cudaStreamCreate",
               __FILE__, __LINE__) ||
      !cuda_ok(cudaEventCreateWithFlags(&ln.done, cudaEventDisableTiming), "cudaEventCreate",
               __FILE__, __LINE__))
    return false;
  for (int i = 1; i < Lane::kSide; ++i)
    if (!cuda_ok(cudaStreamCreateWithFlags(&ln.side[i], cudaStreamNonBlocking), "cudaStreamCreate", __FILE__, __LINE__) ||
        !cuda_ok(cudaEventCreateWithFlags(&ln.side_done[i], cudaEventDisableTiming), "cudaEventCreate", __FILE__, __LINE__))
      return false;
  for (auto &ev : ln.sig)
    if (!cuda_ok(cudaEventCreateWithFlags(&ev, cudaEventDisableTiming), "cudaEventCreate", __FILE__, __LINE__)) return false;
  if (!new_tensor(ln, S, kNet, kNet, kInC, ln.in8, "input")) return false;
  size_t ci = 0;
  Tensor t0, t1, x2, t3, x4, t5, x6, t7, x8, sp, x9, x12, x15, t16, x18, t19, x21;
  const bool par = e->cfg.conv_impl != IRMV_CONV_DIRECT && !getenv("IRMV_NO_RASTER") && !getenv("IRMV_NO_S2_RASTER");
  const bool fused = e->fused_stem && e->cfg.conv_impl != IRMV_CONV_DIRECT;
  const bool par2 = par && getenv("IRMV_S2_DUAL");
  const bool shuffle = e->arch == kArchShuffleKpt;
  if (!new_tensor(ln, S, 320, 320, 16, t0, "m0")) return false;
  if (!shuffle && par && fused && !add_parity_twin(ln, S, t0, true)) return false;
  ln.taps["m0"] = t0;
  add_conv(e, ln, *e->convs[ci++], {{&ln.in8, 0, kInC, 0}}, 640, 640, t0, 0);
  ln.ops.back().cp.out2 = nullptr;
  ln.stem_out = t0;
  if (shuffle) {
    size_t di = 0, bi = 0;
    const Tensor *prev = &ln.stem_out;
    Tensor stage_out[4];
    int hw = 320;
    auto add_dw = [&](const HostDw &d, const Tensor &in, int in_plane0, int H, const Tensor &out) {
      Op op;
      op.kind = Op::DW;
      op.dw.in = in.p + (long long)in_plane0 * in.pstride; op.dw.in_ps = in.pstride;
      op.dw.out = out.p; op.dw.out_ps = out.pstride;
      op.dw.w = d.d_w; op.dw.bias = d.d_b;
      op.dw.planes = d.c / 8; op.dw.B = e->S; op.dw.H = H; op.dw.W = H; op.dw.stride = d.stride; op.dw.rev = 0;
      ln.ops.push_back(op);
    };
    for (int sgi = 0; sgi < 4; ++sgi) {
      const ShuffleStage &st = kShuffleStages[sgi];
      const int h = st.cout / 2, oh = hw / 2;
      Tensor X, Ta, Tb, Tc, T1, T2;
      char nm[8];
      snprintf(nm, sizeof nm, "d%d", sgi + 1);
      if (e->sh_fused && h <= kShuffleFuseMaxH) {
        Tensor XB;
        if (!new_tensor(ln, S, oh, oh, st.cout, X) || (st.units && !new_tensor(ln, S, oh, oh, st.cout, XB))) return false;
        static const int th_force = getenv("IRMV_UNIT_TH") ? atoi(getenv("IRMV_UNIT_TH")) : 0;
        auto pick_th = [&](ShuffleUnitParams q) {
          for (int th : {8, 4, 2}) {
            if (oh % th) continue;
            q.TH = th;
            if (th == th_force || (!th_force && shuffle_unit_ctas_per_sm(q) >= 2)) return th;
          }
          return 1;
        };
        Op op;
        op.kind = Op::SHUF;
        ShuffleUnitParams &q = op.su;
        q.down = 1; q.in = prev->p; q.in_ps = prev->pstride; q.out = X.p; q.out_ps = X.pstride;
        q.B = S; q.H = oh; q.W = oh; q.cin = st.cin; q.h = h; q.first_plane = 0; q.runs = 0;
        q.blob = e->sh_blobs[bi++];
        q.rev = 0; q.num_sms = e->num_sms;
        q.TH = pick_th(q);
        ln.ops.push_back(op);
        ci += 3; di += 2;
        Tensor *cur = &X, *oth = &XB;
        for (int u = 0; u < st.units; ++u) {
          const irmv_engine::ShuffleUnit &su = e->sh_units[sgi][u];
          const int run_planes = su.runs ? (1 << (su.runs - 1)) : h / 8;
          if (su.first_plane != run_planes) { set_error("internal: shuffle unit planes do not start one run in"); return false; }
          Op ob;
          ob.kind = Op::SHUF;
          ShuffleUnitParams &r = ob.su;
          r.down = 0; r.in = cur->p; r.in_ps = cur->pstride; r.out = oth->p; r.out_ps = oth->pstride;
          r.B = S; r.H = oh; r.W = oh; r.cin = h; r.h = h; r.first_plane = su.first_plane; r.runs = su.runs;
          r.blob = e->sh_blobs[bi++];
          r.rev = 0; r.num_sms = e->num_sms;
          r.TH = pick_th(r);
          ln.ops.push_back(ob);
          ci += 2; di += 1;
          std::swap(cur, oth);
        }
        X = *cur;
        X.cmap = e->sh_map[sgi];
        ln.taps[nm] = X;
      } else {
      if (!new_tensor(ln, S, oh, oh, st.cout, X) || !new_tensor(ln, S, oh, oh, st.cin, Ta) ||
          !new_tensor(ln, S, hw, hw, h, Tb) || !new_tensor(ln, S, oh, oh, h, Tc))
        return false;
      X.cmap = e->sh_map[sgi];
      ln.taps[nm] = X;
      add_dw(*e->dws[di++], *prev, 0, hw, Ta);
      add_conv(e, ln, *e->convs[ci++], {{&Ta, 0, st.cin, 0}}, oh, oh, X, 0);
      add_conv(e, ln, *e->convs[ci++], {{prev, 0, st.cin, 0}}, hw, hw, Tb, 0);
      add_dw(*e->dws[di++], Tb, 0, hw, Tc);
      add_conv(e, ln, *e->convs[ci++], {{&Tc, 0, h, 0}}, oh, oh, X, h);
      if (st.units && (!new_tensor(ln, S, oh, oh, h, T1) || !new_tensor(ln, S, oh, oh, h, T2))) return false;
      for (int u = 0; u < st.units; ++u) {
        const irmv_engine::ShuffleUnit &su = e->sh_units[sgi][u];
        add_conv(e, ln, *e->convs[ci++], {{&X, su.first_plane * 8, h, 0}}, oh, oh, T1, 0);
        ln.ops.back().cp.seg[0].runs = su.runs; ln.ops.back().cp.seg[1].runs = su.runs;
        add_dw(*e->dws[di++], T1, 0, oh, T2);
        add_conv(e, ln, *e->convs[ci++], {{&T2, 0, h, 0}}, oh, oh, X, su.first_plane * 8);
        ln.ops.back().cp.out_runs = su.runs;
      }
      }
      stage_out[sgi] = X;
      ln.taps[nm] = X;
      prev = &stage_out[sgi];
      hw = oh;
    }
    for (size_t k = 1; k < ln.ops.size(); ++k)
      if (ln.ops[k].kind == Op::CONV && !ln.ops[k].raster) { set_error("internal: a ShuffleNetV2 1x1 conv does not fit the raster kernel"); return false; }
    if (di != e->dws.size() || ci != 23) { set_error("internal: backbone conv count mismatch"); return false; }
    x4 = stage_out[1]; x6 = stage_out[2]; x8 = stage_out[3];
  } else {
  if (!new_tensor(ln, S, 160, 160, 32, t1, "m1")) return false;
  add_conv(e, ln, *e->convs[ci++], {{&t0, 0, 16, 0}}, 320, 320, t1, 0);
  if (!add_c2f(e, ln, ci, {{&t1, 0, 32, 0}}, 160, 160, 32, 1, true, x2, "m2", par ? 1 : 0)) return false;
  if (!new_tensor(ln, S, 80, 80, 64, t3, "m3")) return false;
  add_conv(e, ln, *e->convs[ci++], {{&x2, 0, 32, 0}}, 160, 160, t3, 0);
  if (!add_c2f(e, ln, ci, {{&t3, 0, 64, 0}}, 80, 80, 64, 2, true, x4, "m4", par2 ? 2 : 0)) return false;
  if (!new_tensor(ln, S, 40, 40, 128, t5, "m5")) return false;
  add_conv(e, ln, *e->convs[ci++], {{&x4, 0, 64, 0}}, 80, 80, t5, 0);
  if (!add_c2f(e, ln, ci, {{&t5, 0, 128, 0}}, 40, 40, 128, 2, true, x6, "m6")) return false;
  if (!new_tensor(ln, S, 20, 20, 256, t7, "m7")) return false;
  add_conv(e, ln, *e->convs[ci++], {{&x6, 0, 128, 0}}, 40, 40, t7, 0);
  if (!add_c2f(e, ln, ci, {{&t7, 0, 256, 0}}, 20, 20, 256, 1, true, x8, "m8")) return false;
  }
  if (!new_tensor(ln, S, 20, 20, 512, sp) || !new_tensor(ln, S, 20, 20, 256, x9, "m9")) return false;
  add_conv(e, ln, *e->convs[ci++], {{&x8, 0, 256, 0}}, 20, 20, sp, 0);
  {
    Op op; op.kind = Op::POOL; op.pool_buf = sp.p; op.pH = 20; op.pW = 20; op.pC = 128; op.pStride = sp.pstride;
    ln.ops.push_back(op);
  }
  add_conv(e, ln, *e->convs[ci++], {{&sp, 0, 512, 0}}, 20, 20, x9, 0);
  if (!add_c2f(e, ln, ci, {{&x9, 0, 256, 1}, {&x6, 0, 128, 0}}, 40, 40, 128, 1, false, x12, "m12")) return false;
  if (!add_c2f(e, ln, ci, {{&x12, 0, 128, 1}, {&x4, 0, 64, 0}}, 80, 80, 64, 1, false, x15, "m15", par2 ? 2 : 0)) return false;
  ln.ops.back().signal = 0;
  if (!new_tensor(ln, S, 40, 40, 64, t16, "m16")) return false;
  add_conv(e, ln, *e->convs[ci++], {{&x15, 0, 64, 0}}, 80, 80, t16, 0);
  if (!add_c2f(e, ln, ci, {{&t16, 0, 64, 0}, {&x12, 0, 128, 0}}, 40, 40, 128, 1, false, x18, "m18")) return false;
  ln.ops.back().signal = 1;
  if (!new_tensor(ln, S, 20, 20, 128, t19, "m19")) return false;
  add_conv(e, ln, *e->convs[ci++], {{&x18, 0, 128, 0}}, 40, 40, t19, 0);
  if (!add_c2f(e, ln, ci, {{&t19, 0, 128, 0}, {&x9, 0, 256, 0}}, 20, 20, 256, 1, false, x21, "m21")) return false;
  ln.ops.back().signal = 2;
  const Tensor *feat[3] = {&x15, &x18, &x21};
  const int hw[3] = {80, 40, 20};
  for (int i = 0; i < 3; ++i) {
    Tensor h0, hb, hc, bo, co;
    char nb[8], ncn[8];
    snprintf(nb, sizeof nb, "box%d", i);
    snprintf(ncn, sizeof ncn, "cls%d", i);
    if (!new_tensor(ln, S, hw[i], hw[i], 128, h0) || !new_tensor(ln, S, hw[i], hw[i], 64, hb) ||
        !new_tensor(ln, S, hw[i], hw[i], 64, hc) || !new_tensor(ln, S, hw[i], hw[i], 64, bo, nb) ||
        !new_tensor(ln, S, hw[i], hw[i], kClsPad, co, ncn))
      return false;
    const int s_box = i < 2 ? 1 + 2 * i : 0, s_cls = i < 2 ? 2 + 2 * i : 5;
    add_conv(e, ln, *e->convs[ci++], {{feat[i], 0, feat[i]->C, 0}}, hw[i], hw[i], h0, 0);
    ln.ops.back().stream = s_box; ln.ops.back().wait = i; ln.ops.back().signal = 3 + i;
    add_conv(e, ln, *e->convs[ci++], {{&h0, 0, 64, 0}}, hw[i], hw[i], hb, 0);
    ln.ops.back().stream = s_box;
    add_conv(e, ln, *e->convs[ci++], {{&hb, 0, 64, 0}}, hw[i], hw[i], bo, 0);
    ln.ops.back().stream = s_box;
    add_conv(e, ln, *e->convs[ci++], {{&h0, 64, 64, 0}}, hw[i], hw[i], hc, 0);
    ln.ops.back().stream = s_cls; ln.ops.back().wait = 3 + i;
    add_conv(e, ln, *e->convs[ci++], {{&hc, 0, 64, 0}}, hw[i], hw[i], co, 0);
    ln.ops.back().stream = s_cls;
    ln.heads.box[i] = bo.p; ln.heads.box_ps[i] = bo.pstride;
    ln.heads.cls[i] = co.p; ln.heads.cls_ps[i] = co.pstride;
    ln.heads.padded = 1;
  }
  if (e->pose)
    for (int i = 0; i < 3; ++i) {
      Tensor k0, k1, ko;
      char nk[8];
      snprintf(nk, sizeof nk, "kpt%d", i);
      if (!new_tensor(ln, S, hw[i], hw[i], 16, k0) || !new_tensor(ln, S, hw[i], hw[i], 16, k1) ||
          !new_tensor(ln, S, hw[i], hw[i], 16, ko, nk))
        return false;
      add_conv(e, ln, *e->convs[ci++], {{feat[i], 0, feat[i]->C, 0}}, hw[i], hw[i], k0, 0);
      ln.ops.back().stream = 6 + i; ln.ops.back().wait = i;
      add_conv(e, ln, *e->convs[ci++], {{&k0, 0, 16, 0}}, hw[i], hw[i], k1, 0);
      ln.ops.back().stream = 6 + i;
      add_conv(e, ln, *e->convs[ci++], {{&k1, 0, 16, 0}}, hw[i], hw[i], ko, 0);
      ln.ops.back().stream = 6 + i;
      ln.kpt[i] = ko.p;
    }
  if (ci != e->convs.size()) { set_error("internal: conv count mismatch"); return false; }
  fuse_tails(e, ln);
  if (!lane_alloc(ln, (void **)&ln.nms.boxes, (size_t)S * kNumAnchors * 16) ||
      !lane_alloc(ln, (void **)&ln.nms.keys, (size_t)S * kNumAnchors * e->nc * 8) ||
      !lane_alloc(ln, (void **)&ln.nms.counts, (size_t)S * 4))
    return false;
  ln.det.init(S, e->cfg.max_det);
  if (!lane_alloc(ln, (void **)&ln.src_word, sizeof(void *))) return false;
  const size_t slots = (size_t)S * e->cfg.max_det;
  {
    auto up = [](size_t v, size_t a) { return (v + a - 1) & ~(a - 1); };
    const size_t o_rvec = up(ln.det.bytes, 16), o_tvec = o_rvec + slots * 24, o_ok = o_tvec + slots * 24;
    const size_t o_arm = up(o_ok + slots, 64), o_kpt = o_arm + slots * sizeof(ArmorOut);
    const size_t o_quat = up(o_kpt + slots * 32, 64), o_dist = o_quat + slots * 32;
    uint8_t *blk = nullptr;
    if (!lane_alloc(ln, (void **)&blk, o_dist + slots * 4)) return false;
    ln.det.dev = blk;
    ln.pnp_rvec = reinterpret_cast<double *>(blk + o_rvec);
    ln.pnp_tvec = reinterpret_cast<double *>(blk + o_tvec);
    ln.pnp_ok = blk + o_ok;
    ln.armors = reinterpret_cast<ArmorOut *>(blk + o_arm);
    ln.kpts = reinterpret_cast<float *>(blk + o_kpt);
    ln.pnp_quat = reinterpret_cast<double *>(blk + o_quat);
    ln.pnp_dist = reinterpret_cast<float *>(blk + o_dist);
  }
  if (!lane_alloc(ln, (void **)&ln.pnp_pts, slots * 32) || !lane_alloc(ln, (void **)&ln.pnp_centers, slots * 8)) return false;
  for (auto &ev : ln.stage_ev)
    if (!cuda_ok(cudaEventCreate(&ev), "cudaEventCreate", __FILE__, __LINE__)) return false;
  Tensor bt; bt.p = reinterpret_cast<__half *>(ln.nms.boxes); bt.H = 1; bt.W = kNumAnchors; bt.C = 4; bt.pstride = 0;
  ln.taps["boxes"] = bt;
  return true;
}

int issue_replay(irmv_engine *e, Lane &ln, int n, cudaStream_t st, int *launches,
                 bool stage_events = false, std::vector<cudaEvent_t> *op_events = nullptr) {
  int cnt = 0;
  auto op_mark = [&]() {
    if (!op_events) return;
    cudaEvent_t ev = nullptr;
    cudaEventCreate(&ev);
    cudaEventRecord(ev, st);
    op_events->push_back(ev);
  };
  auto mark = [&](int i) -> int {
    if (stage_events) IRMV_CUDA(cudaEventRecord(ln.stage_ev[i], st));
    return 0;
  };
  if (mark(0)) return 1;
  PreprocessParams pp{};
  pp.src = nullptr; pp.src_indirect = ln.src_word; pp.dst = ln.in8.p; pp.rotated = ln.rotated;
  pp.n = n; pp.src_w = e->cfg.src_width; pp.src_h = e->cfg.src_height; pp.frame0 = 0;
  pp.chan_order = e->cfg.chan_order; pp.rotate180 = e->cfg.rotate180;
  pp.resize_mode = e->cfg.resize_mode; pp.quantize_u8 = e->cfg.quantize_u8;
  const bool fused = e->fused_stem && e->cfg.conv_impl != IRMV_CONV_DIRECT;
  if (fused) IRMV_CUDA(launch_stem(pp, e->d_stem_w, e->d_stem_b, e->d_stem_tab, ln.stem_out.parity_only ? nullptr : ln.stem_out.p, ln.stem_out.pstride, ln.stem_out.pp, ln.stem_out.pp_stride, st));
  else IRMV_CUDA(launch_preprocess(pp, st));
  cnt += 1 + (ln.rotated ? 1 : 0);
  if (mark(1)) return 1;
  op_mark();
  static const bool pingpong = !getenv("IRMV_NO_PINGPONG");
  static const int branch_max = getenv("IRMV_BRANCH_MAX") ? atoi(getenv("IRMV_BRANCH_MAX")) : 64;
  const bool branched = n <= branch_max && !stage_events && !op_events && e->cfg.conv_impl != IRMV_CONV_DIRECT;
  unsigned side_used = 0;
  const cudaStream_t trunk = st;
  int seq = 0;
  bool first = true;
  for (auto &op : ln.ops) {
    if (first && fused) { first = false; continue; }
    first = false;
    ++seq;
    st = trunk;
    if (branched) {
      if (op.stream > 0) { st = ln.side[op.stream]; side_used |= 1u << op.stream; }
      if (op.wait >= 0) IRMV_CUDA(cudaStreamWaitEvent(st, ln.sig[op.wait], 0));
    }
    if (op.kind == Op::CONV) {
      ConvParams p = op.cp;
      p.B = n;
      p.rev_tiles = pingpong ? (seq & 1) : 0;
      if (e->cfg.conv_impl == IRMV_CONV_DIRECT) IRMV_CUDA(launch_conv_direct(p, st));
      else if (op.raster) IRMV_CUDA(launch_conv_raster(p, e->num_sms, st));
      else IRMV_CUDA(launch_conv_tc(p, e->num_sms, st));
    } else if (op.kind == Op::SHUF) {
      ShuffleUnitParams q = op.su;
      q.B = n;
      q.rev = pingpong ? (seq & 1) : 0;
      IRMV_CUDA(launch_shuffle_unit(q, st));
    } else if (op.kind == Op::DW) {
      DwParams d = op.dw;
      d.B = n;
      d.rev = pingpong ? (seq & 1) : 0;
      IRMV_CUDA(launch_dwconv3x3(d, st));
    } else {
      IRMV_CUDA(launch_sppf_pool(op.pool_buf, n, op.pH, op.pW, op.pStride, op.pC, st));
    }
    ++cnt;
    if (branched && op.signal >= 0) IRMV_CUDA(cudaEventRecord(ln.sig[op.signal], st));
    op_mark();
    if (getenv("IRMV_SYNC_EACH")) {
      cudaError_t ce = cudaStreamSynchronize(st);
      if (ce != cudaSuccess) {
        char buf[256];
        snprintf(buf, sizeof buf, "op %d (%s k=%d s=%d cin=%d cout=%d H=%d) failed: %s", cnt - 2,
                 op.kind == Op::POOL ? "pool" : (op.kind == Op::DW ? "dw" : (op.kind == Op::SHUF ? "shuffle-unit" : (op.raster ? "raster" : "gather"))), op.cp.k, op.cp.stride, op.cp.cin,
                 op.cp.cout, op.cp.H, cudaGetErrorString(ce));
        set_error(buf);
        return 1;
      }
    }
  }
  st = trunk;
  for (int i = 1; i < Lane::kSide; ++i)
    if (side_used & (1u << i)) {
      IRMV_CUDA(cudaEventRecord(ln.side_done[i], ln.side[i]));
      IRMV_CUDA(cudaStreamWaitEvent(st, ln.side_done[i], 0));
    }
  if (mark(2)) return 1;
  IRMV_CUDA(launch_decode(ln.heads, n, e->nc, e->cfg.score_thr, ln.nms, nullptr, st)); ++cnt;
  DetOut out{ln.det.num(), ln.det.boxes(), ln.det.scores(), ln.det.classes(), ln.det.index()};
  IRMV_CUDA(launch_nms(ln.nms, n, kNumAnchors, e->nc, e->cfg.iou_thr, e->cfg.max_det, out, st)); ++cnt;
  if (e->pose) {
    const int total = n * e->cfg.max_det;
    kpts_from_dets_kernel<<<(total + 127) / 128, 128, 0, st>>>(ln.det.num(), ln.det.index(), n, e->cfg.max_det, e->nc,
                                                              ln.kpt[0], ln.kpt[1], ln.kpt[2], ln.kpts);
    IRMV_CUDA(cudaGetLastError());
    ++cnt;
  }
  if (mark(3)) return 1;
  if (e->armors_on) {
    int pad_x, pad_y, new_w, new_h;
    letterbox_geometry(e->cfg.src_width, e->cfg.src_height, e->cfg.resize_mode, &pad_x, &pad_y, &new_w, &new_h);
    ArmorParams ap{};
    ap.src = nullptr; ap.src_indirect = ln.src_word;
    ap.n = n; ap.src_w = e->cfg.src_width; ap.src_h = e->cfg.src_height;
    ap.chan_order = e->cfg.chan_order; ap.rotate180 = e->cfg.rotate180;
    ap.num = ln.det.num(); ap.boxes = ln.det.boxes(); ap.scores = ln.det.scores(); ap.classes = ln.det.classes();
    ap.max_det = e->cfg.max_det;
    ap.box_sx = (float)e->cfg.src_width / new_w; ap.box_sy = (float)e->cfg.src_height / new_h;
    ap.box_px = (float)pad_x; ap.box_py = (float)pad_y;
    const irmv_armor_params &q = e->armor_prm;
    ap.binary_threshold = q.binary_threshold;
    ap.min_ratio = q.light_min_ratio; ap.max_ratio = q.light_max_ratio; ap.max_angle = q.light_max_angle;
    ap.min_small = q.min_small_center_distance; ap.max_small = q.max_small_center_distance;
    ap.min_large = q.min_large_center_distance; ap.max_large = q.max_large_center_distance;
    ap.out = ln.armors; ap.slot_locks = reinterpret_cast<int *>(ln.armor_scratch); ap.scratch = ln.armor_scratch + 64;
    ap.scratch_words_per_cta = armors_scratch_words_per_cta(e->cfg.src_width, e->cfg.src_height);
    ap.grid = armors_grid(e->num_sms);
    IRMV_CUDA(launch_extract_armors(ap, st)); ++cnt;
    if (e->pnp_on) {
      const int total = n * e->cfg.max_det;
      IRMV_CUDA(launch_quads_from_armors(ln.armors, total, e->corner_sx, e->corner_sy, ln.pnp_pts, ln.pnp_centers, st));
      PnpOut po{ln.pnp_rvec, ln.pnp_tvec, ln.pnp_ok, ln.pnp_quat, nullptr, nullptr, nullptr, ln.pnp_dist, ln.pnp_centers};
      IRMV_CUDA(launch_pnp(e->pnp_c, ln.pnp_pts, total, 0, po, st));
      IRMV_CUDA(launch_mask_pose_ok(ln.armors, total, ln.pnp_ok, st));
      cnt += 3;
// ... 876 lines not shown
double irmv_extract_armors_last_device_ms(void) { return g_armors_ms; }
int irmv_extract_armors_last_profile(unsigned long long out[8]) {
  if (!out) return 1;
  for (int i = 0; i < 8; ++i) out[i] = g_armors_prof[i];
  return 0;
}

int irmv_engine_has_keypoints(irmv_engine *e) { return e && e->pose ? 1 : 0; }

int irmv_engine_fetch_keypoints(irmv_engine *e, int ticket, int nframes, float *kpts) {
  if (!e || !kpts || nframes < 1 || nframes > e->cfg.max_batch) { set_error("bad argument"); return 1; }
  if (!e->pose) { set_error("the weight file has no keypoint branch"); return 2; }
  const size_t md = e->cfg.max_det, B = e->cfg.max_batch;
  const uint8_t *h = result_block(e, ticket);
  if (!h) return 2;
  const float *src = reinterpret_cast<const float *>(h + kpts_offset(B, md));
  int pad_x, pad_y, new_w, new_h;
  letterbox_geometry(e->cfg.src_width, e->cfg.src_height, e->cfg.resize_mode, &pad_x, &pad_y, &new_w, &new_h);
  const float sx = (float)e->cfg.src_width / new_w, sy = (float)e->cfg.src_height / new_h;
  const float px = (float)pad_x, py = (float)pad_y;
  for (size_t i = 0; i < (size_t)nframes * md * 4; ++i) {
    kpts[2 * i] = (src[2 * i] - px) * sx;
    kpts[2 * i + 1] = (src[2 * i + 1] - py) * sy;
  }
  return 0;
}

int irmv_extract_armors(const uint8_t *frames, int frames_on_device, int nframes, int src_w, int src_h, int chan_order,
                        int rotate180, const irmv_bbox *boxes, const int *counts, int max_det,
                        const irmv_armor_params *prm, int device, irmv_armor *out) {
  if (!frames || !boxes || !counts || !out || nframes < 1 || max_det < 1 || src_w < 2 || src_h < 2) { set_error("bad argument"); return 1; }
  irmv_armor_params q;
  if (prm) q = *prm; else irmv_armor_params_default(&q);
  IRMV_CUDA(cudaSetDevice(device));
  cudaDeviceProp prop;
  IRMV_CUDA(cudaGetDeviceProperties(&prop, device));
  const size_t fb = (size_t)src_w * src_h * (chan_order >= 2 ? 1 : 3), slots = (size_t)nframes * max_det;
  uint8_t *d_frames = nullptr;
  int32_t *d_num = nullptr, *d_cls = nullptr;
  float *d_boxes = nullptr, *d_scores = nullptr;
  ArmorOut *d_out = nullptr;
  uint32_t *d_scratch = nullptr;
  std::vector<float> hb(slots * 4, 0.f), hs(slots, 0.f);
  std::vector<int32_t> hc(slots, 0);
  for (size_t i = 0; i < slots; ++i) {
    for (int k = 0; k < 4; ++k) hb[i * 4 + k] = boxes[i].xyxy[k];
    hs[i] = boxes[i].score; hc[i] = boxes[i].class_id;
  }
  const int grid = armors_grid(prop.multiProcessorCount);
  const size_t wpc = armors_scratch_words_per_cta(src_w, src_h), wtotal = armors_scratch_total_words(src_w, src_h, grid);
  int rc = 0;
  auto body = [&]() -> int {
    if (!frames_on_device) {
      IRMV_CUDA(dev_malloc((void **)&d_frames, fb * nframes));
      IRMV_CUDA(cudaMemcpy(d_frames, frames, fb * nframes, cudaMemcpyHostToDevice));
    }
    IRMV_CUDA(dev_malloc((void **)&d_num, (size_t)nframes * 4));
    IRMV_CUDA(dev_malloc((void **)&d_cls, slots * 4));
    IRMV_CUDA(dev_malloc((void **)&d_boxes, slots * 16));
    IRMV_CUDA(dev_malloc((void **)&d_scores, slots * 4));
    IRMV_CUDA(dev_malloc((void **)&d_out, slots * sizeof(ArmorOut)));
    IRMV_CUDA(dev_malloc((void **)&d_scratch, wtotal * 4));
    IRMV_CUDA(cudaMemset(d_scratch, 0, 256));
    IRMV_CUDA(cudaMemcpy(d_num, counts, (size_t)nframes * 4, cudaMemcpyHostToDevice));
    IRMV_CUDA(cudaMemcpy(d_cls, hc.data(), slots * 4, cudaMemcpyHostToDevice));
    IRMV_CUDA(cudaMemcpy(d_boxes, hb.data(), slots * 16, cudaMemcpyHostToDevice));
    IRMV_CUDA(cudaMemcpy(d_scores, hs.data(), slots * 4, cudaMemcpyHostToDevice));
    IRMV_CUDA(cudaMemset(d_out, 0, slots * sizeof(ArmorOut)));
    ArmorParams ap{};
    ap.src = frames_on_device ? frames : d_frames; ap.src_indirect = nullptr;
    ap.n = nframes; ap.src_w = src_w; ap.src_h = src_h; ap.chan_order = chan_order; ap.rotate180 = rotate180;
    ap.num = d_num; ap.boxes = d_boxes; ap.scores = d_scores; ap.classes = d_cls; ap.max_det = max_det;
    ap.box_sx = 1.f; ap.box_sy = 1.f; ap.box_px = 0.f; ap.box_py = 0.f;
    ap.binary_threshold = q.binary_threshold;
    ap.min_ratio = q.light_min_ratio; ap.max_ratio = q.light_max_ratio; ap.max_angle = q.light_max_angle;
    ap.min_small = q.min_small_center_distance; ap.max_small = q.max_small_center_distance;
    ap.min_large = q.min_large_center_distance; ap.max_large = q.max_large_center_distance;
    ap.out = d_out; ap.slot_locks = reinterpret_cast<int *>(d_scratch); ap.scratch = d_scratch + 64;
    ap.scratch_words_per_cta = wpc; ap.grid = grid;
    unsigned long long *d_prof = nullptr;
    if (getenv("IRMV_ARMOR_PROF")) {
      IRMV_CUDA(dev_malloc((void **)&d_prof, 64));
      IRMV_CUDA(cudaMemset(d_prof, 0, 64));
    }
    ap.prof = d_prof;
    cudaEvent_t e0 = nullptr, e1 = nullptr;
    IRMV_CUDA(cudaEventCreate(&e0));
    IRMV_CUDA(cudaEventCreate(&e1));
    IRMV_CUDA(cudaEventRecord(e0, nullptr));
    IRMV_CUDA(launch_extract_armors(ap, nullptr));
    IRMV_CUDA(cudaEventRecord(e1, nullptr));
    IRMV_CUDA(cudaDeviceSynchronize());
    float ms = 0.f;
    IRMV_CUDA(cudaEventElapsedTime(&ms, e0, e1));
    g_armors_ms = ms;
    cudaEventDestroy(e0); cudaEventDestroy(e1);
    if (d_prof) {
      IRMV_CUDA(cudaMemcpy(g_armors_prof, d_prof, 64, cudaMemcpyDeviceToHost));
      cudaFree(d_prof);
    }
    IRMV_CUDA(cudaMemcpy(out, d_out, slots * sizeof(ArmorOut), cudaMemcpyDeviceToHost));
    return 0;
  };
  rc = body();
  cudaFree(d_frames); cudaFree(d_num); cudaFree(d_cls); cudaFree(d_boxes); cudaFree(d_scores); cudaFree(d_out); cudaFree(d_scratch);
  return rc;
}

int irmv_engine_profile_stages(irmv_engine *e, const uint8_t *frames_dev, int nframes, float ms[5]) {
  if (!e || !frames_dev || !ms || nframes < 1) { set_error("bad argument"); return 1; }
  IRMV_CUDA(cudaSetDevice(e->cfg.device));
  Lane &ln = e->lanes[0];
  const int n = nframes < e->S ? nframes : e->S;
  IRMV_CUDA(cudaDeviceSynchronize());
  set_src_kernel<<<1, 1, 0, ln.stream>>>(ln.src_word, frames_dev);
  IRMV_CUDA(cudaGetLastError());
  int launches = 0;
  if (int rc = issue_replay(e, ln, n, ln.stream, &launches, true)) return rc;
  IRMV_CUDA(cudaStreamSynchronize(ln.stream));
  for (int i = 0; i < 4; ++i) IRMV_CUDA(cudaEventElapsedTime(&ms[i], ln.stage_ev[i], ln.stage_ev[i + 1]));
  IRMV_CUDA(cudaEventElapsedTime(&ms[4], ln.stage_ev[0], ln.stage_ev[4]));
  return n;
}

int irmv_engine_profile_ops(irmv_engine *e, const uint8_t *frames_dev, int nframes, float *ms, int cap) {
  if (!e || !frames_dev || !ms || nframes < 1) { set_error("bad argument"); return -1; }
  cudaSetDevice(e->cfg.device);
  Lane &ln = e->lanes[0];
  const int n = nframes < e->S ? nframes : e->S;
  cudaDeviceSynchronize();
  set_src_kernel<<<1, 1, 0, ln.stream>>>(ln.src_word, frames_dev);
  std::vector<cudaEvent_t> evs;
  int launches = 0;
  if (issue_replay(e, ln, n, ln.stream, &launches, false, &evs)) return -1;
  if (cudaStreamSynchronize(ln.stream) != cudaSuccess) { set_error("profile_ops: replay failed"); return -1; }
  int k = 0;
  for (size_t i = 1; i < evs.size() && k < cap; ++i, ++k) cudaEventElapsedTime(&ms[k], evs[i - 1], evs[i]);
  for (auto ev : evs) cudaEventDestroy(ev);
  return k;
}

int irmv_engine_describe_ops(irmv_engine *e, char *buf, int cap) {
  if (!e || !buf || cap < 1) return -1;
  std::string out;
  bool first = true;
  const bool fused = e->fused_stem && e->cfg.conv_impl != IRMV_CONV_DIRECT;
  for (auto &o : e->lanes[0].ops) {
    if (first && fused) { first = false; continue; }
    first = false;
    char line[160];
    if (o.kind == Op::POOL) snprintf(line, sizeof line, "pool\n");
    else if (o.kind == Op::DW) snprintf(line, sizeof line, "dw %d %d %d\n", o.dw.stride, o.dw.planes * 8, o.dw.H / o.dw.stride);
    else if (o.kind == Op::SHUF) snprintf(line, sizeof line, "unit %d %d %d %d %d\n", o.su.down, o.su.cin, o.su.h, o.su.H, o.su.TH);
    else snprintf(line, sizeof line, "conv %d %d %d %d %d %d %d\n", o.cp.k, o.cp.stride, o.cp.cin, o.cp.cout, o.cp.OH,
                  o.raster ? 1 : 0, o.cp.tail_w ? o.cp.tail_cout : 0);
    out += line;
  }
  if ((int)out.size() + 1 > cap) { set_error("buffer too small"); return -1; }
  memcpy(buf, out.c_str(), out.size() + 1);
  return (int)out.size();
}

int irmv_engine_describe_plans(irmv_engine *e, int nframes, char *buf, int cap) {
  if (!e || !buf || cap < 1 || nframes < 1) return -1;
  std::string out;
  bool first = true;
  const bool fused = e->fused_stem && e->cfg.conv_impl != IRMV_CONV_DIRECT;
  const int n = nframes < e->S ? nframes : e->S;
  for (auto &o : e->lanes[0].ops) {
    if (first && fused) { first = false; continue; }
    first = false;
    char line[200];
    if (o.kind == Op::POOL) { out += "pool\n"; continue; }
    if (o.kind == Op::DW) { snprintf(line, sizeof line, "dw %d %d %d\n", o.dw.stride, o.dw.planes * 8, o.dw.H / o.dw.stride); out += line; continue; }
    if (o.kind == Op::SHUF) { snprintf(line, sizeof line, "unit %d %d %d %d %d\n", o.su.down, o.su.cin, o.su.h, o.su.H, o.su.TH); out += line; continue; }
    ConvParams p = o.cp;
    p.B = n;
    int info[8];
    if (o.raster && conv_raster_plan_info(p, e->num_sms, info))
      snprintf(line, sizeof line, "raster %d %d %d %d %d %d %d %d %d %d %d %d %d %d %d\n", p.k, p.stride, p.cin, p.cout, p.OH,
               info[0], info[1], info[2], info[3], info[4], info[5], info[6], p.act, p.res ? 1 : 0, info[7]);
    else
      snprintf(line, sizeof line, "gather %d %d %d %d %d\n", p.k, p.stride, p.cin, p.cout, p.OH);
    out += line;
  }
  if ((int)out.size() + 1 > cap) { set_error("buffer too small"); return -1; }
  memcpy(buf, out.c_str(), out.size() + 1);
  return (int)out.size();
}

int irmv_engine_trace_conv(irmv_engine *e, int op_index, int nframes, long long *out, int cap_tiles, float *kernel_ms) {
  if (!e || !out || cap_tiles < 1) { set_error("bad argument"); return -1; }
  cudaSetDevice(e->cfg.device);
  Lane &ln = e->lanes[0];
  int ci = -1;
  Op *op = nullptr;
  for (auto &o : ln.ops) if (o.kind == Op::CONV && ++ci == op_index) { op = &o; break; }
  if (!op) { set_error("no such conv"); return -1; }
  long long *d = nullptr;
  dev_malloc((void **)&d, (size_t)(cap_tiles + 16) * 64);
  cudaMemset(d, 0, (size_t)(cap_tiles + 16) * 64);
  ConvParams p = op->cp;
  p.B = nframes < e->S ? nframes : e->S;
  p.trace = d; p.trace_cap = cap_tiles;
  if (const char *dbg = getenv("IRMV_TC_DEBUG")) p.sync_mode = atoi(dbg);
  cudaDeviceSynchronize();
  cudaEventRecord(ln.stage_ev[0], ln.stream);
  if (op->raster) launch_conv_raster(p, e->num_sms, ln.stream); else launch_conv_tc(p, e->num_sms, ln.stream);
  cudaEventRecord(ln.stage_ev[1], ln.stream);
  cudaError_t ce = cudaStreamSynchronize(ln.stream);
  if (kernel_ms) cudaEventElapsedTime(kernel_ms, ln.stage_ev[0], ln.stage_ev[1]);
  cudaMemcpy(out, d, (size_t)(cap_tiles + 16) * 64, cudaMemcpyDeviceToHost);
  cudaFree(d);
  if (ce != cudaSuccess) { set_error(cudaGetErrorString(ce)); return -1; }
  int M = p.B * p.OH * p.OW, tiles = (M + 127) / 128;
  if (op->raster) return cap_tiles;
  int per_cta = (tiles + (tiles < e->num_sms ? tiles : e->num_sms) - 1) / (tiles < e->num_sms ? tiles : e->num_sms);
  return per_cta < cap_tiles ? per_cta : cap_tiles;
}

int irmv_preprocess(const uint8_t *src, int n, int src_w, int src_h, int chan_order, int rotate180,
                    int resize_mode, int quantize_u8, uint16_t *dst, uint8_t *rotated, int device) {
  if (!src || !dst || n < 1) { set_error("bad argument"); return 1; }
  IRMV_CUDA(cudaSetDevice(device));
  const size_t fb = (size_t)src_w * src_h * (chan_order >= 2 ? 1 : 3);
  const size_t ob = (size_t)pr_pixels(n, kNet, kNet) * kInC * 2;
  uint8_t *ds = nullptr, *dr = nullptr;
  __half *dd = nullptr;
  IRMV_CUDA(dev_malloc((void **)&ds, fb * n));
  IRMV_CUDA(dev_malloc((void **)&dd, ob));
  IRMV_CUDA(cudaMemset(dd, 0, ob));
  if (rotated) IRMV_CUDA(dev_malloc((void **)&dr, (size_t)src_w * src_h * 3 * n));
  IRMV_CUDA(cudaMemcpy(ds, src, fb * n, cudaMemcpyHostToDevice));
  PreprocessParams pp{};
  pp.src = ds; pp.dst = dd; pp.rotated = dr; pp.n = n; pp.src_w = src_w; pp.src_h = src_h;
  pp.chan_order = chan_order; pp.rotate180 = rotate180; pp.resize_mode = resize_mode; pp.quantize_u8 = quantize_u8;
  cudaError_t ce = launch_preprocess(pp, 0);
  if (ce == cudaSuccess) ce = cudaDeviceSynchronize();
  std::vector<uint16_t> tmp(ob / 2);
  if (ce == cudaSuccess) ce = cudaMemcpy(tmp.data(), dd, ob, cudaMemcpyDeviceToHost);
  if (ce == cudaSuccess && rotated) ce = cudaMemcpy(rotated, dr, (size_t)src_w * src_h * 3 * n, cudaMemcpyDeviceToHost);
  cudaFree(ds); cudaFree(dd); if (dr) cudaFree(dr);
  IRMV_CUDA(ce);
  for (int b = 0; b < n; ++b)
    for (int y = 0; y < kNet; ++y)
      memcpy(dst + (((size_t)b * kNet + y) * kNet) * kInC, tmp.data() + (size_t)pr_index(b, y, 0, kNet, kNet) * kInC,
             (size_t)kNet * kInC * 2);
  return 0;
}

static int alloc_nms(int n, int A, int nc, int max_det, NmsScratch &sc, DetPack &dp) {
  IRMV_CUDA(dev_malloc((void **)&sc.boxes, (size_t)n * A * 16));
  IRMV_CUDA(dev_malloc((void **)&sc.keys, (size_t)n * A * nc * 8));
  IRMV_CUDA(dev_malloc((void **)&sc.counts, (size_t)n * 4));
  IRMV_CUDA(cudaMemset(sc.counts, 0, (size_t)n * 4));
  dp.init(n, max_det);
  IRMV_CUDA(dev_malloc((void **)&dp.dev, dp.bytes));
  IRMV_CUDA(cudaMemset(dp.dev, 0, dp.bytes));
  return 0;
}

int irmv_nms(const float *boxes, const float *scores, int n, int A, int nc, float score_thr,
             float iou_thr, int max_det, int32_t *num_dets, float *det_boxes, float *det_scores,
             int32_t *det_classes, int32_t *det_index, int device) {
  if (!boxes || !scores || !num_dets || n < 1 || A < 1 || nc < 1 || max_det < 1) { set_error("bad argument"); return 1; }
  IRMV_CUDA(cudaSetDevice(device));
  NmsScratch sc{};
  DetPack dp;
  if (int rc = alloc_nms(n, A, nc, max_det, sc, dp)) return rc;
  float *ds = nullptr;
  IRMV_CUDA(dev_malloc((void **)&ds, (size_t)n * A * nc * 4));
  IRMV_CUDA(cudaMemcpy(sc.boxes, boxes, (size_t)n * A * 16, cudaMemcpyHostToDevice));
  IRMV_CUDA(cudaMemcpy(ds, scores, (size_t)n * A * nc * 4, cudaMemcpyHostToDevice));
  cudaError_t ce = launch_score_filter(ds, n, A, nc, score_thr, sc, 0);
  DetOut out{dp.num(), dp.boxes(), dp.scores(), dp.classes(), dp.index()};
  if (ce == cudaSuccess) ce = launch_nms(sc, n, A, nc, iou_thr, max_det, out, 0);
  if (ce == cudaSuccess) ce = cudaDeviceSynchronize();
  std::vector<uint8_t> host(dp.bytes);
  if (ce == cudaSuccess) ce = cudaMemcpy(host.data(), dp.dev, dp.bytes, cudaMemcpyDeviceToHost);
  cudaFree(sc.boxes); cudaFree(sc.keys); cudaFree(sc.counts); cudaFree(dp.dev); cudaFree(ds);
  IRMV_CUDA(ce);
  memcpy(num_dets, host.data(), (size_t)n * 4);
  if (det_boxes) memcpy(det_boxes, host.data() + dp.off_boxes(), (size_t)n * max_det * 16);
  if (det_scores) memcpy(det_scores, host.data() + dp.off_scores(), (size_t)n * max_det * 4);
  if (det_classes) memcpy(det_classes, host.data() + dp.off_classes(), (size_t)n * max_det * 4);
  if (det_index) memcpy(det_index, host.data() + dp.off_index(), (size_t)n * max_det * 4);
  return 0;
}

int irmv_decode(const uint16_t *box, const uint16_t *cls, int n, float *boxes, float *scores, int device) {
  if (!box || !cls || !boxes || !scores || n < 1) { set_error("bad argument"); return 1; }
  IRMV_CUDA(cudaSetDevice(device));
  const int nc = IRMV_NUM_CLASSES;
  NmsScratch sc{};
  DetPack dp;
  if (int rc = alloc_nms(n, kNumAnchors, nc, 1, sc, dp)) return rc;
  const int cnt[3] = {6400, 1600, 400}, off[3] = {0, 6400, 8000};
  HeadPtrs h{};
  __half *db[3], *dc[3];
  float *dscores = nullptr;
  IRMV_CUDA(dev_malloc((void **)&dscores, (size_t)n * kNumAnchors * nc * 4));
  for (int s = 0; s < 3; ++s) {
    IRMV_CUDA(dev_malloc((void **)&db[s], (size_t)n * cnt[s] * 64 * 2));
    IRMV_CUDA(dev_malloc((void **)&dc[s], (size_t)n * cnt[s] * kClsPad * 2));
    for (int f = 0; f < n; ++f) {
      IRMV_CUDA(cudaMemcpy(db[s] + (size_t)f * cnt[s] * 64, box + ((size_t)f * kNumAnchors + off[s]) * 64,
                           (size_t)cnt[s] * 64 * 2, cudaMemcpyHostToDevice));
      IRMV_CUDA(cudaMemcpy(dc[s] + (size_t)f * cnt[s] * kClsPad, cls + ((size_t)f * kNumAnchors + off[s]) * kClsPad,
// ... 175 lines not shown
```

### irmv_detection_b200/engine.py

```python
from __future__ import annotations

import ctypes as C
import enum
import os
from dataclasses import dataclass
from typing import List, Optional, Sequence, Tuple

import numpy as np

from . import _lib as L


class ArmorClass(enum.IntEnum):
    B1 = 0; B2 = 1; B3 = 2; B4 = 3; B5 = 4; BO = 5; BS = 6
    R1 = 7; R2 = 8; R3 = 9; R4 = 10; R5 = 11; RO = 12; RS = 13
    UNKNOWN = 14


@dataclass
class bbox:
    xyxy: Tuple[float, float, float, float]
    score: float
    class_id: ArmorClass

# ... 52 lines not shown
        if not p:
            raise L.IrmvError("bad slot")
        buf = (C.c_uint8 * self.frame_bytes).from_address(p)
        shape = (self.src_image_size[1], self.src_image_size[0]) + ((3,) if self.channels == 3 else ())
        return np.frombuffer(buf, np.uint8).reshape(shape)

    def detect(self, slot: int = 0) -> List[bbox]:
        n = C.c_int(0)
        L.check(self._lib.irmv_engine_detect(self._h, slot, self._out, self.max_det, C.byref(n)), "irmv_engine_detect")
        self._slot = slot
        return self._to_list(0, n.value)

    def get_rotated_image(self, slot: Optional[int] = None) -> np.ndarray:
        slot = self._slot if slot is None else slot
        out = np.empty((self.src_image_size[1], self.src_image_size[0], 3), np.uint8)
        L.check(self._lib.irmv_engine_rotated_image(self._h, slot, out.ctypes.data), "irmv_engine_rotated_image")
        return out

    def get_rotated_view(self, slot: Optional[int] = None) -> np.ndarray:
        slot = self._slot if slot is None else slot
        p = C.c_void_p()
        L.check(self._lib.irmv_engine_rotated_view(self._h, slot, C.byref(p)), "irmv_engine_rotated_view")
        n = self.src_image_size[0] * self.src_image_size[1] * 3
        buf = (C.c_uint8 * n).from_address(p.value)
        return np.frombuffer(buf, np.uint8).reshape(self.src_image_size[1], self.src_image_size[0], 3)

    def get_profiling_time(self) -> float:
        return float(self._lib.irmv_engine_profile_ms(self._h))

    def detect_batch(self, frames: np.ndarray) -> List[List[bbox]]:
        frames = np.ascontiguousarray(frames, np.uint8)
        n = frames.shape[0]
        if frames[0].size != self.frame_bytes:
            raise ValueError("frame size does not match the engine's src_image_size")
        L.check(self._lib.irmv_engine_detect_batch(self._h, frames.ctypes.data, 0, n, self._out, self._counts),
                "irmv_engine_detect_batch")
        return [self._to_list(f, self._counts[f]) for f in range(n)]

    def detect_batch_arrays(self, frames: np.ndarray):
        frames = np.ascontiguousarray(frames, np.uint8)
        n = frames.shape[0]
        L.check(self._lib.irmv_engine_detect_batch(self._h, frames.ctypes.data, 0, n, self._out, self._counts),
                "irmv_engine_detect_batch")
        dt = np.dtype([("xyxy", np.float32, 4), ("score", np.float32), ("class_id", np.int32)])
        dets = np.frombuffer(self._out, dtype=dt, count=n * self.max_det).reshape(n, self.max_det)
        return np.frombuffer(self._counts, dtype=np.int32, count=n), dets

    def submit_batch(self, frames: np.ndarray) -> int:
        if not frames.flags.c_contiguous or frames.dtype != np.uint8:
            raise ValueError("submit_batch needs a C-contiguous uint8 array")
        n = frames.shape[0]
        if frames[0].size != self.frame_bytes:
            raise ValueError("frame size does not match the engine's src_image_size")
        t = C.c_int(0)
        L.check(self._lib.irmv_engine_submit_batch(self._h, frames.ctypes.data, n, C.byref(t)), "irmv_engine_submit_batch")
        self._ticket_n[t.value % 3] = n
        return t.value

    def collect_arrays(self, ticket: int, poses: bool = False):
        n = self._ticket_n[ticket % 3]
        rv = tv = ok = None
        if poses:
            rv = np.empty((n, self.max_det, 3)); tv = np.empty((n, self.max_det, 3))
            ok = np.empty((n, self.max_det), np.uint8)
        L.check(self._lib.irmv_engine_collect(self._h, ticket, self._out, self._counts,
                                              rv.ctypes.data if poses else None, tv.ctypes.data if poses else None,
                                              ok.ctypes.data if poses else None), "irmv_engine_collect")
        dt = np.dtype([("xyxy", np.float32, 4), ("score", np.float32), ("class_id", np.int32)])
        dets = np.frombuffer(self._out, dtype=dt, count=n * self.max_det).reshape(n, self.max_det)
        counts = np.frombuffer(self._counts, dtype=np.int32, count=n)
        return (counts, dets, rv, tv, ok.astype(bool)) if poses else (counts, dets)

    def detect_batch_device(self, dev_ptr: int, n: int) -> List[List[bbox]]:
        L.check(self._lib.irmv_engine_detect_batch(self._h, C.c_void_p(dev_ptr), 1, n, self._out, self._counts),
                "irmv_engine_detect_batch")
        return [self._to_list(f, self._counts[f]) for f in range(n)]

    def enqueue_batch_device(self, dev_ptr: int, n: int) -> None:
        L.check(self._lib.irmv_engine_enqueue_batch(self._h, C.c_void_p(dev_ptr), n), "irmv_engine_enqueue_batch")

    def sync(self) -> float:
        L.check(self._lib.irmv_engine_sync(self._h), "irmv_engine_sync")
        return float(self._lib.irmv_engine_last_device_ms(self._h))

    def fetch(self, n: int) -> List[List[bbox]]:
        L.check(self._lib.irmv_engine_fetch(self._h, n, self._out, self._counts), "irmv_engine_fetch")
        return [self._to_list(f, self._counts[f]) for f in range(n)]

    def last_device_ms(self) -> float:
        return float(self._lib.irmv_engine_last_device_ms(self._h))

    def copy_bytes(self) -> Tuple[int, int]:
        a, b = C.c_ulonglong(0), C.c_ulonglong(0)
        L.check(self._lib.irmv_engine_copy_bytes(self._h, C.byref(a), C.byref(b)), "irmv_engine_copy_bytes")
        return int(a.value), int(b.value)

    def kernel_launches(self, n: int) -> int:
        return int(self._lib.irmv_engine_kernel_launches(self._h, n))

    def enable_pnp(self, camera_matrix, dist_coeffs, corner_scale=(1.0, 1.0)) -> None:
        K = (C.c_double * 9)(*[float(v) for v in camera_matrix])
        D = (C.c_double * 5)(*[float(v) for v in list(dist_coeffs)[:5]])
        L.check(self._lib.irmv_engine_enable_pnp(self._h, K, D, float(corner_scale[0]), float(corner_scale[1])),
                "irmv_engine_enable_pnp")

    def fetch_poses(self, n: int):
        rv = np.empty((n, self.max_det, 3)); tv = np.empty((n, self.max_det, 3))
        ok = np.empty((n, self.max_det), np.uint8)
        L.check(self._lib.irmv_engine_fetch_poses(self._h, n, rv.ctypes.data, tv.ctypes.data, ok.ctypes.data),
                "irmv_engine_fetch_poses")
        return rv, tv, ok.astype(bool)

    def fetch_armor_poses(self, n: int, ticket: int = -1) -> np.ndarray:
        out = np.zeros((n, self.max_det), POSE_DTYPE)
        L.check(self._lib.irmv_engine_fetch_armor_poses(self._h, ticket, n, out.ctypes.data), "irmv_engine_fetch_armor_poses")
        return out

    def has_keypoints(self) -> bool:
        return bool(self._lib.irmv_engine_has_keypoints(self._h))

    def fetch_keypoints(self, n: int, ticket: int = -1) -> np.ndarray:
        out = np.zeros((n, self.max_det, 4, 2), np.float32)
        L.check(self._lib.irmv_engine_fetch_keypoints(self._h, ticket, n, out.ctypes.data), "irmv_engine_fetch_keypoints")
        return out

    def enable_armors(self, **params) -> None:
        prm = armor_params(**params)
        L.check(self._lib.irmv_engine_enable_armors(self._h, C.byref(prm)), "irmv_engine_enable_armors")

    def fetch_armors(self, n: int, ticket: int = -1) -> np.ndarray:
        out = np.zeros((n, self.max_det), ARMOR_DTYPE)
        L.check(self._lib.irmv_engine_fetch_armors(self._h, ticket, n, out.ctypes.data), "irmv_engine_fetch_armors")
        return out

    def check_padding(self) -> int:
        bad = C.c_longlong(-1)
        L.check(self._lib.irmv_debug_check_padding(self._h, C.byref(bad)), "irmv_debug_check_padding")
        return int(bad.value)

    def describe_ops(self):
        buf = C.create_string_buffer(16384)
        if self._lib.irmv_engine_describe_ops(self._h, buf, 16384) < 0:
            L.check(1, "irmv_engine_describe_ops")
        ops = []
        for line in buf.value.decode().splitlines():
            f = line.split()
            if f[0] == "pool":
                ops.append({"kind": "pool"})
            elif f[0] == "dw":
                ops.append({"kind": "dw", "s": int(f[1]), "c": int(f[2]), "hw": int(f[3])})
            elif f[0] == "unit":
                ops.append({"kind": "unit", "down": bool(int(f[1])), "cin": int(f[2]), "h": int(f[3]), "hw": int(f[4]), "rows_per_cta": int(f[5])})
            else:
                k, s, cin, cout, hw, raster, tail = (int(v) for v in f[1:])
                ops.append({"kind": "conv", "k": k, "s": s, "cin": cin, "cout": cout, "hw": hw, "raster": bool(raster),
                            "tail_cout": tail})
        return ops

    def describe_plans(self, n: int):
        buf = C.create_string_buffer(32768)
        if self._lib.irmv_engine_describe_plans(self._h, n, buf, 32768) < 0:
            L.check(1, "irmv_engine_describe_plans")
        out = []
        for line in buf.value.decode().splitlines():
            f = line.split()
            out.append((f[0],) + tuple(int(v) for v in f[1:]))
        return out

    def profile_stages(self, dev_ptr: int, n: int):
        ms = (C.c_float * 5)()
        k = self._lib.irmv_engine_profile_stages(self._h, C.c_void_p(dev_ptr), n, C.byref(ms))
        if k <= 0:
            L.check(1, "irmv_engine_profile_stages")
        return k, dict(zip(("preprocess", "conv", "decode_nms", "pnp", "total"), [float(v) for v in ms]))

    def read_tensor(self, name: str) -> np.ndarray:
        dims = (C.c_int32 * 5)()
        L.check(self._lib.irmv_engine_read_tensor(self._h, name.encode(), None, 0, C.byref(dims)), "read_tensor")
        b, h, w, c, es = list(dims)
        out = np.empty((b, h, w, c), np.float32 if es == 4 else np.float16)
        L.check(self._lib.irmv_engine_read_tensor(self._h, name.encode(), out.ctypes.data, out.nbytes, C.byref(dims)),
                "read_tensor")
        return out

    def kept_indices(self, frame: int = 0) -> np.ndarray:
        idx = np.empty(self.max_det, np.int32)
        n = C.c_int(0)
        L.check(self._lib.irmv_engine_read_kept_indices(self._h, frame, idx.ctypes.data, self.max_det, C.byref(n)),
                "read_kept_indices")
        return idx[: n.value].copy()

    def _to_list(self, frame: int, k: int) -> List[bbox]:
        out = []
        base = frame * self.max_det
        for i in range(k):
            b = self._out[base + i]
            out.append(bbox(tuple(b.xyxy), float(b.score), ArmorClass(int(b.class_id))))
        return out

    def close(self) -> None:
        if getattr(self, "_h", None) and self._h.value:
            self._lib.irmv_engine_destroy(self._h)
            self._h = C.c_void_p()

    def __del__(self):
        try:
            self.close()
        except Exception:
            pass


class PnPSolver:

    def __init__(self, camera_matrix: Sequence[float], dist_coeffs: Sequence[float], device: int = 0):
        self._lib = L.lib()
        K = (C.c_double * 9)(*[float(v) for v in camera_matrix])
        D = (C.c_double * 5)(*[float(v) for v in list(dist_coeffs)[:5]])
        self._h = C.c_void_p()
        L.check(self._lib.irmv_pnp_create(K, D, device, C.byref(self._h)), "irmv_pnp_create")

    def solvePnP(self, points) -> Tuple[bool, np.ndarray, np.ndarray]:
        pts = (C.c_float * 8)(*np.asarray(points, np.float32).reshape(8))
        r = (C.c_double * 3)()
        t = (C.c_double * 3)()
        ok = C.c_int(0)
        L.check(self._lib.irmv_pnp_solve(self._h, pts, r, t, C.byref(ok)), "irmv_pnp_solve")
        return bool(ok.value), np.array(r[:]).reshape(3, 1), np.array(t[:]).reshape(3, 1)

    def solve_batch(self, points: np.ndarray, large_armor: bool = False, extended: bool = False):
        pts = np.ascontiguousarray(points, np.float32).reshape(-1, 8)
        n = pts.shape[0]
        rv = np.empty((n, 3)); tv = np.empty((n, 3)); ok = np.empty(n, np.uint8)
        if not extended:
            L.check(self._lib.irmv_pnp_solve_batch(self._h, pts.ctypes.data, n, 0, int(large_armor),
                                                   rv.ctypes.data, tv.ctypes.data, ok.ctypes.data), "irmv_pnp_solve_batch")
            return rv, tv, ok.astype(bool)
        q = np.empty((n, 4)); rv2 = np.empty((n, 3)); tv2 = np.empty((n, 3)); e = np.empty((n, 2))
        L.check(self._lib.irmv_pnp_solve_batch_ex(self._h, pts.ctypes.data, n, 0, int(large_armor), rv.ctypes.data,
                                                  tv.ctypes.data, ok.ctypes.data, q.ctypes.data, rv2.ctypes.data,
                                                  tv2.ctypes.data, e.ctypes.data), "irmv_pnp_solve_batch_ex")
        return rv, tv, ok.astype(bool), q, rv2, tv2, e

    def solve_batch_device(self, dev_ptr: int, n: int, rv: np.ndarray, tv: np.ndarray, ok: np.ndarray,
                           large_armor: bool = False) -> float:
        L.check(self._lib.irmv_pnp_solve_batch(self._h, C.c_void_p(dev_ptr), n, 1, int(large_armor),
                                               rv.ctypes.data, tv.ctypes.data, ok.ctypes.data), "irmv_pnp_solve_batch")
        return float(self._lib.irmv_pnp_last_device_ms(self._h))

    def last_device_ms(self) -> float:
        return float(self._lib.irmv_pnp_last_device_ms(self._h))

    def set_refine_lm(self, max_iters: int = 20) -> None:
        L.check(self._lib.irmv_pnp_set_refine_lm(self._h, int(max_iters)), "irmv_pnp_set_refine_lm")

    def calculateDistanceToCenter(self, image_point) -> float:
        return float(self._lib.irmv_pnp_distance_to_center(self._h, float(image_point[0]), float(image_point[1])))

    def close(self) -> None:
        if getattr(self, "_h", None) and self._h.value:
            self._lib.irmv_pnp_destroy(self._h)
            self._h = C.c_void_p()

    def __del__(self):
        try:
            self.close()
        except Exception:
            pass


ARMOR_DTYPE = np.dtype([("pts", np.float32, (4, 2)), ("center", np.float32, 2), ("score", np.float32),
                        ("class_id", np.int32), ("size", np.int32), ("valid", np.int32)])
POSE_DTYPE = np.dtype([("position", np.float64, 3), ("orientation", np.float64, 4), ("rvec", np.float64, 3),
                       ("distance_to_image_center", np.float32), ("ok", np.int32)])
BBOX_DTYPE = np.dtype([("xyxy", np.float32, 4), ("score", np.float32), ("class_id", np.int32)])


def armor_params(**kw) -> "L.ArmorParams":
    prm = L.ArmorParams()
    L.check(L.lib().irmv_armor_params_default(C.byref(prm)), "irmv_armor_params_default")
    for k, v in kw.items():
        if not hasattr(prm, k):
            raise TypeError(f"unknown armor parameter {k}")
        setattr(prm, k, v)
    return prm


def extract_armors(frames: np.ndarray, boxes: np.ndarray, counts: np.ndarray, chan_order: int = L.CH_PASSTHROUGH,
                   rotate180: bool = True, device: int = 0, **params) -> np.ndarray:
    frames = np.ascontiguousarray(frames, np.uint8)
    n, H, W = frames.shape[:3]
    return extract_armors_ptr(frames.ctypes.data, False, n, W, H, boxes, counts, chan_order, rotate180, device, **params)


def extract_armors_ptr(ptr: int, on_device: bool, n: int, W: int, H: int, boxes: np.ndarray, counts: np.ndarray,
                       chan_order: int = L.CH_PASSTHROUGH, rotate180: bool = True, device: int = 0, **params) -> np.ndarray:
    boxes = np.ascontiguousarray(boxes, BBOX_DTYPE)
    counts = np.ascontiguousarray(counts, np.int32)
    max_det = boxes.shape[1]
    out = np.zeros((n, max_det), ARMOR_DTYPE)
    prm = armor_params(**params)
    L.check(L.lib().irmv_extract_armors(C.c_void_p(ptr), int(on_device), n, W, H, chan_order, int(rotate180),
                                        boxes.ctypes.data, counts.ctypes.data, max_det, C.byref(prm), device,
                                        out.ctypes.data), "irmv_extract_armors")
    return out


def extract_armors_last_device_ms() -> float:
    return float(L.lib().irmv_extract_armors_last_device_ms())

# ... 42 lines not shown
```

Before: 54480.

## Fuse back-to-back C2f bottleneck 3x3 convs into one raster kernel

Adds a HEAD mode to the tcgen05 raster conv kernel so the first 3x3 conv of a C2f bottleneck is computed on the fly inside the second conv's kernel. Each CTA processes a contiguous band of tiles, runs the first conv's MMA into a separate TMEM region, and applies SiLU in its epilogue into a shared-memory sliding window with a mirrored halo. The second conv then reads its A operand from that window. This removes a kernel launch and the global write and re-read of the intermediate activation. In exchange it needs more shared memory and TMEM, applies only to large feature maps, and adds a more complex pipeline with halo recomputation at band edges.

Result: no change. 54620 (median of 6 runs) (+0.3%).

```diff
diff --git a/irmv_detection_b200/csrc/common.cuh b/irmv_detection_b200/csrc/common.cuh
--- a/irmv_detection_b200/csrc/common.cuh
+++ b/irmv_detection_b200/csrc/common.cuh
@@ -114,6 +114,8 @@
   int trace_cap;
   const __half *w_raster_split;
   int split_ways;
+  const __half *head_w;
+  const float *head_bias;
 };
 cudaError_t launch_conv_direct(const ConvParams &p, cudaStream_t s);
 cudaError_t launch_conv_tc(const ConvParams &p, int num_sms, cudaStream_t s);
diff --git a/irmv_detection_b200/csrc/conv_raster.cu b/irmv_detection_b200/csrc/conv_raster.cu
--- a/irmv_detection_b200/csrc/conv_raster.cu
+++ b/irmv_detection_b200/csrc/conv_raster.cu
@@ -19,6 +19,8 @@
   uint64_t mid_full, mid_empty;
   uint64_t ext_full[2], ext_empty[2];
   uint64_t tail_full[2], tail_empty[2];
+  uint64_t head_full[2], head_empty[2];
+  uint64_t win_full;
   uint64_t bfull;
   uint32_t tmem_base;
   uint32_t pad;
@@ -123,6 +125,9 @@
   int rev;
   int tmem_tail0;
   int nsplit;
+  int lead, win_head, win_pix, tmem_head0;
+  uint32_t off_win, off_bh, off_hbias, bh_bytes, head_idesc;
+  uint32_t tap_w[9];
 };
 
 __device__ __forceinline__ void st_shared_v4(uint32_t addr, const uint4 &v) {
@@ -195,7 +200,13 @@
   }
 }
 
-template <int R, int NEPI, bool ACT, int RES, int TAIL>
+__device__ __forceinline__ uint4 ld_shared_v4(uint32_t addr) {
+  uint4 v;
+  asm volatile("ld.shared.v4.b32 {%0, %1, %2, %3}, [%4];" : "=r"(v.x), "=r"(v.y), "=r"(v.z), "=r"(v.w) : "r"(addr) : "memory");
+  return v;
+}
+
+template <int R, int NEPI, bool ACT, int RES, int TAIL, bool HEAD = false>
 __global__ void __launch_bounds__((NEPI + 2) * 32, NEPI == 8 ? 2 : 1) conv_raster_kernel(const __grid_constant__ RArgs a) {
   constexpr int NTHREADS = (NEPI + 2) * 32;
   constexpr int TMA_WARP = NEPI, MMA_WARP = NEPI + 1;
@@ -208,6 +219,9 @@
   uint8_t *sExt = smem + a.off_ext;
   uint8_t *sBt = smem + a.off_bt;
   float *s_tb = reinterpret_cast<float *>(smem + a.off_tbias);
+  uint8_t *sWin = smem + a.off_win;
+  uint8_t *sBh = smem + a.off_bh;
+  float *s_hab = reinterpret_cast<float *>(smem + a.off_hbias);
   Bars *bars = reinterpret_cast<Bars *>(smem + a.off_bars);
   const int tid = threadIdx.x, warp = tid >> 5, lane = tid & 31;
   const int npad = p.npad;
@@ -215,6 +229,8 @@
   const int bid = nsplit > 1 ? (int)(blockIdx.x / (unsigned)nsplit) : (int)blockIdx.x;
   const int gsz = nsplit > 1 ? (int)(gridDim.x / (unsigned)nsplit) : (int)gridDim.x;
   const int split = nsplit > 1 ? (int)(blockIdx.x % (unsigned)nsplit) : 0;
+  const int band0 = HEAD ? (int)((long long)bid * a.num_tiles / gsz) : 0;
+  const int nband = HEAD ? (int)((long long)(bid + 1) * a.num_tiles / gsz) - band0 : 0;
   const float *const bias_g = p.bias + split * npad;
   const uint8_t *const w_g = reinterpret_cast<const uint8_t *>(p.w_raster) + (size_t)split * a.b_bytes;
   long long *trow = (p.trace && tid == 0 && (blockIdx.x == 0 || blockIdx.x == gridDim.x - 1))
@@ -230,6 +246,8 @@
   for (int i = tid; i < npad; i += NTHREADS) s_hb[i] = ACT ? 0.5f * bias_g[i] : bias_g[i];
   if (TAIL)
     for (int i = tid; i < p.tail_npad; i += NTHREADS) s_tb[i] = TAIL == 2 ? 0.5f * p.tail_bias[i] : p.tail_bias[i];
+  if (HEAD)
+    for (int i = tid; i < p.cin; i += NTHREADS) s_hab[i] = 0.5f * p.head_bias[i];
   if (tid == 0) {
     for (int s = 0; s < a.stages; ++s) {
       mbar_init(&bars->full[s], 1);
@@ -253,6 +271,13 @@
     for (int i = 0; i < 2; ++i) {
       mbar_init(&bars->tail_full[i], 1);
       mbar_init(&bars->tail_empty[i], NEPI);
+    }
+    if (HEAD) {
+      for (int i = 0; i < 2; ++i) {
+        mbar_init(&bars->head_full[i], 1);
+        mbar_init(&bars->head_empty[i], NEPI);
+      }
+      mbar_init(&bars->win_full, NEPI);
     }
     asm volatile("fence.mbarrier_init.release.cluster;" ::: "memory");
   }
@@ -268,12 +293,17 @@
   if (trow) trow[1] = clock64();
   if (warp == TMA_WARP && !a.b_stream && elect_one()) {
     const uint32_t bar = smem_u32(&bars->bfull), sB_u = smem_u32(sB);
-    mbar_expect_tx(bar, a.b_bytes + (TAIL ? a.bt_bytes : 0u));
+    mbar_expect_tx(bar, a.b_bytes + (TAIL ? a.bt_bytes : 0u) + (HEAD ? a.bh_bytes : 0u));
     for (uint32_t off = 0; off < a.b_bytes; off += 65536u) {
       const uint32_t n = a.b_bytes - off < 65536u ? a.b_bytes - off : 65536u;
       bulk_g2s(sB_u + off, w_g + off, n, bar);
     }
     if (TAIL) bulk_g2s(smem_u32(sBt), p.tail_w, a.bt_bytes, bar);
+    if (HEAD) {
+      const uint8_t *hw = reinterpret_cast<const uint8_t *>(p.head_w);
+      for (uint32_t off = 0; off < a.bh_bytes; off += 65536u)
+        bulk_g2s(smem_u32(sBh) + off, hw + off, a.bh_bytes - off < 65536u ? a.bh_bytes - off : 65536u, bar);
+    }
   }
   asm volatile("griddepcontrol.wait;" ::: "memory");
 
@@ -352,9 +382,7 @@
       __syncwarp();
       if (lane == 0) mbar_arrive(&bars->tail_empty[tb]);
     };
-    int it = 0, prev_tile = -1;
-    for (int tseq = bid; tseq < num_tiles; tseq += gsz, ++it) {
-      const int tile = a.rev ? num_tiles - 1 - tseq : tseq;
+    auto main_epilogue = [&](int it, int tile) {
       const int buf = it & 1;
       const uint32_t aph = (uint32_t)(it >> 1) & 1u;
       const bool tr = trace && blockIdx.x == 0 && tid == 0 && it < trace_cap;
@@ -432,10 +460,66 @@
         if (TAIL) mbar_arrive(&bars->mid_full);
       }
       if (tr) trace[it * 8 + 7] = clock64();
+    };
+    if constexpr (HEAD) {
+      const int hcin = p.cin;
+      const int hshift = 31 - __clz(hcin >> 4), hmask = (hcin >> 4) - 1;
+      const int q_begin = a.q_begin, win_head = a.win_head;
+      const uint32_t win_plane = (uint32_t)a.win_pix * 16u, mirror_off = (uint32_t)(2 * TM) * 16u;
+      const uint4 z = make_uint4(0, 0, 0, 0);
+      auto head_epilogue = [&](int k) {
+        const int hb = k & 1;
+        mbar_wait_warp(&bars->head_full[hb], (uint32_t)(k >> 1) & 1u, lane);
+        if (k >= 2) mbar_wait_warp(&bars->tmem_full[k & 1], (uint32_t)((k - 2) >> 1) & 1u, lane);
+        tc_fence_after();
+        const int q_tile = q_lane + (band0 - 1 + k) * TM + a.lead;
+        const uint32_t hcol = lane_base + (uint32_t)(a.tmem_head0 + hb * R * hcin);
+        const uint32_t wlane = smem_u32(sWin) + (uint32_t)(hb * TM + ew * 32 + lane) * 16u;
+        for (int w = sub; w < (R << hshift); w += NSUB) {
+          const int r = w >> hshift, c0 = (w & hmask) << 4;
+          uint32_t v[16];
+          tc_ld16(hcol + (uint32_t)(r * hcin + c0), v);
+          const int qi = q_tile + r * 128;
+          bool ok = qi >= q_begin && qi < q_end;
+          if (ok) {
+            const uint32_t row = (uint32_t)(((uint64_t)(uint32_t)qi * mul_wp) >> 34);
+            const int x = qi - (int)row * Wp;
+            const uint32_t img = (uint32_t)(((uint64_t)row * mul_hp1) >> 34);
+            ok = x < W && (int)row - (int)img * Hp1 != 0;
+          }
+          const uint32_t wa = wlane + (uint32_t)((c0 >> 3) * a.win_pix + r * 128) * 16u;
+          tc_ld_wait();
+          if (ok) epi_chunk<true, 0, true>(v, s_hab + c0, nullptr, 0, nullptr, 0, z, z, wa, win_plane);
+          else st_shared_zero2(wa, win_plane);
+          if (hb == 0 && r * 128 + ew * 32 + lane < win_head) {
+            st_shared_v4(wa + mirror_off, ld_shared_v4(wa));
+            st_shared_v4(wa + win_plane + mirror_off, ld_shared_v4(wa + win_plane));
+          }
+        }
+        asm volatile("fence.proxy.async.shared::cta;" ::: "memory");
+        tc_fence_before();
+        __syncwarp();
+        if (lane == 0) {
+          mbar_arrive(&bars->head_empty[hb]);
+          mbar_arrive(&bars->win_full);
+        }
+      };
+      head_epilogue(0);
+      for (int i = 0; i < nband; ++i) {
+        head_epilogue(i + 1);
+        if (i >= 1) main_epilogue(i - 1, band0 + i - 1);
+      }
+      main_epilogue(nband - 1, band0 + nband - 1);
+    } else {
+      int it = 0, prev_tile = -1;
+      for (int tseq = bid; tseq < num_tiles; tseq += gsz, ++it) {
+        const int tile = a.rev ? num_tiles - 1 - tseq : tseq;
+        main_epilogue(it, tile);
+        if (TAIL && it > 0) tail_epilogue(it - 1, prev_tile);
+        prev_tile = tile;
+      }
       if (TAIL && it > 0) tail_epilogue(it - 1, prev_tile);
-      prev_tile = tile;
-    }
-    if (TAIL && it > 0) tail_epilogue(it - 1, prev_tile);
+    }
   } else if (warp == TMA_WARP) {
     if (elect_one()) {
       const uint32_t sA_u = smem_u32(sA), sB_u = smem_u32(sB);
@@ -460,7 +544,7 @@
       };
       auto issue_main = [&](int tile, int itl) {
         const bool tr = p.trace && blockIdx.x == 0 && itl < p.trace_cap;
-        const long long qlo = (long long)a.q_begin + (long long)tile * a.TM - a.halo_front;
+        const long long qlo = (long long)a.q_begin + (long long)tile * a.TM + (HEAD ? a.lead : 0) - a.halo_front;
         if (tr) p.trace[itl * 8 + 1] = clock64();
         const uint32_t bar = smem_u32(&bars->full[s]);
         mbar_expect_tx(bar, tile_tx);
@@ -498,6 +582,11 @@
             }
           }
           if (!progressed) __nanosleep(64);
+        }
+      } else if (HEAD) {
+        for (int i = 0; i <= nband; ++i) {
+          mbar_wait(&bars->empty[s], ph ^ 1u);
+          issue_main(band0 - 1 + i, i);
         }
       } else {
         for (int tseq = bid; tseq < a.num_tiles; tseq += gsz, ++itl) {
@@ -564,61 +653,119 @@
       }
       __syncwarp();
     };
-    for (int tile = bid; tile < a.num_tiles; tile += gsz, ++it) {
-      const int buf = it & 1;
-      const uint32_t aph = (uint32_t)(it >> 1) & 1u;
-      const bool tr = p.trace && blockIdx.x == 0 && lane == 0 && it < p.trace_cap;
-      if (tr) p.trace[it * 8 + 3] = clock64();
-      mbar_wait_warp(&bars->tmem_empty[buf], aph ^ 1u, lane);
-      mbar_wait_warp(&bars->full[s], ph, lane);
-      tc_fence_after();
-      if (tr) p.trace[it * 8 + 4] = clock64();
-      const uint32_t tmem_d0 = tmem_base + (uint32_t)(buf * R * npad);
-      const uint32_t a_stage_lo = a_lo0 + (uint32_t)s * a_stage_u;
-      if (!a.b_stream) {
+    if constexpr (HEAD) {
+      const int hcin = p.cin;
+      const uint32_t bh_lo0 = desc_lo(smem_u32(sBh), (uint32_t)hcin * 16u);
+      const uint32_t win_lo0 = desc_lo(smem_u32(sWin), (uint32_t)a.win_pix * 16u);
+      const uint32_t bh_pair_u = 2u * (uint32_t)hcin, bh_tap_u = (uint32_t)(hcin * hcin) >> 3;
+      const uint32_t win_pair_u = 2u * (uint32_t)a.win_pix;
+      auto issue_head = [&](int k) {
+        const int hb = k & 1;
+        mbar_wait_warp(&bars->head_empty[hb], ((uint32_t)(k >> 1) & 1u) ^ 1u, lane);
+        mbar_wait_warp(&bars->full[s], ph, lane);
+        tc_fence_after();
         if (elect_one()) {
-          uint32_t acc = 0;
-          uint32_t bl_t = b_lo0;
+          const uint32_t td0 = tmem_base + (uint32_t)(a.tmem_head0 + hb * R * hcin);
+          const uint32_t a_stage_lo = a_lo0 + (uint32_t)s * a_stage_u;
+          uint32_t acc = 0, bl_t = bh_lo0;
+          for (int t = 0; t < nchunks; ++t, bl_t += bh_tap_u) {
+            uint32_t al = a_stage_lo + a.tap_a[t], bl = bl_t;
+            for (int j = 0; j < pairs; ++j, al += a_pair_u, bl += bh_pair_u) {
+#pragma unroll
+              for (int r = 0; r < R; ++r)
+                tc_mma_f16(td0 + (uint32_t)(r * hcin), al + (uint32_t)(r * 128), kDescHi, bl, kDescHi, a.head_idesc, acc);
+              acc = 1;
+            }
+          }
+          tc_commit(&bars->empty[s]);
+          tc_commit(&bars->head_full[hb]);
+        }
+        __syncwarp();
+        if (++s == a.stages) { s = 0; ph ^= 1u; }
+      };
+      issue_head(0);
+      issue_head(1);
+      mbar_wait_warp(&bars->win_full, 0u, lane);
+      for (int i = 0; i < nband; ++i) {
+        const int buf = i & 1;
+        if (i + 2 <= nband) issue_head(i + 2);
+        mbar_wait_warp(&bars->win_full, (uint32_t)(i + 1) & 1u, lane);
+        mbar_wait_warp(&bars->tmem_empty[buf], ((uint32_t)(i >> 1) & 1u) ^ 1u, lane);
+        tc_fence_after();
+        if (elect_one()) {
+          const uint32_t tmem_d0 = tmem_base + (uint32_t)(buf * R * npad);
+          const uint32_t w_lo = win_lo0 + (uint32_t)(buf * a.TM);
+          uint32_t acc = 0, bl_t = b_lo0;
           for (int t = 0; t < nchunks; ++t, bl_t += b_tap_u) {
-            uint32_t al = a_stage_lo + a.tap_a[t], bl = bl_t;
-            for (int j = 0; j < pairs; ++j, al += a_pair_u, bl += b_pair_u) {
+            uint32_t al = w_lo + a.tap_w[t], bl = bl_t;
+            for (int j = 0; j < pairs; ++j, al += win_pair_u, bl += b_pair_u) {
 #pragma unroll
               for (int r = 0; r < R; ++r)
                 tc_mma_f16(tmem_d0 + (uint32_t)(r * npad), al + (uint32_t)(r * 128), kDescHi, bl, kDescHi, a.idesc, acc);
               acc = 1;
             }
           }
-          tc_commit(&bars->empty[s]);
           tc_commit(&bars->tmem_full[buf]);
         }
         __syncwarp();
-      } else {
-        for (int t = 0; t < nchunks; ++t) {
-          mbar_wait_warp(&bars->bw_full[bs], bph, lane);
-          tc_fence_after();
+      }
+    } else {
+      for (int tile = bid; tile < a.num_tiles; tile += gsz, ++it) {
+        const int buf = it & 1;
+        const uint32_t aph = (uint32_t)(it >> 1) & 1u;
+        const bool tr = p.trace && blockIdx.x == 0 && lane == 0 && it < p.trace_cap;
+        if (tr) p.trace[it * 8 + 3] = clock64();
+        mbar_wait_warp(&bars->tmem_empty[buf], aph ^ 1u, lane);
+        mbar_wait_warp(&bars->full[s], ph, lane);
+        tc_fence_after();
+        if (tr) p.trace[it * 8 + 4] = clock64();
+        const uint32_t tmem_d0 = tmem_base + (uint32_t)(buf * R * npad);
+        const uint32_t a_stage_lo = a_lo0 + (uint32_t)s * a_stage_u;
+        if (!a.b_stream) {
           if (elect_one()) {
-            uint32_t al = a_stage_lo + a.tap_a[t], bl = b_lo0 + (uint32_t)bs * b_tap_u;
-            for (int j = 0; j < pairs; ++j, al += a_pair_u, bl += b_pair_u) {
-#pragma unroll
-              for (int r = 0; r < R; ++r)
-                tc_mma_f16(tmem_d0 + (uint32_t)(r * npad), al + (uint32_t)(r * 128), kDescHi, bl, kDescHi, a.idesc,
-                           (t | j) != 0 ? 1u : 0u);
+            uint32_t acc = 0;
+            uint32_t bl_t = b_lo0;
+            for (int t = 0; t < nchunks; ++t, bl_t += b_tap_u) {
+              uint32_t al = a_stage_lo + a.tap_a[t], bl = bl_t;
+              for (int j = 0; j < pairs; ++j, al += a_pair_u, bl += b_pair_u) {
+  #pragma unroll
+                for (int r = 0; r < R; ++r)
+                  tc_mma_f16(tmem_d0 + (uint32_t)(r * npad), al + (uint32_t)(r * 128), kDescHi, bl, kDescHi, a.idesc, acc);
+                acc = 1;
+              }
             }
-            tc_commit(&bars->bw_empty[bs]);
-            if (t == nchunks - 1) {
-              tc_commit(&bars->empty[s]);
-              tc_commit(&bars->tmem_full[buf]);
-            }
+            tc_commit(&bars->empty[s]);
+            tc_commit(&bars->tmem_full[buf]);
           }
           __syncwarp();
-          if (++bs == a.b_stages) { bs = 0; bph ^= 1u; }
-        }
+        } else {
+          for (int t = 0; t < nchunks; ++t) {
+            mbar_wait_warp(&bars->bw_full[bs], bph, lane);
+            tc_fence_after();
+            if (elect_one()) {
+              uint32_t al = a_stage_lo + a.tap_a[t], bl = b_lo0 + (uint32_t)bs * b_tap_u;
+              for (int j = 0; j < pairs; ++j, al += a_pair_u, bl += b_pair_u) {
+  #pragma unroll
+                for (int r = 0; r < R; ++r)
+                  tc_mma_f16(tmem_d0 + (uint32_t)(r * npad), al + (uint32_t)(r * 128), kDescHi, bl, kDescHi, a.idesc,
+                             (t | j) != 0 ? 1u : 0u);
+              }
+              tc_commit(&bars->bw_empty[bs]);
+              if (t == nchunks - 1) {
+                tc_commit(&bars->empty[s]);
+                tc_commit(&bars->tmem_full[buf]);
+              }
+            }
+            __syncwarp();
+            if (++bs == a.b_stages) { bs = 0; bph ^= 1u; }
+          }
+        }
+        if (tr) p.trace[it * 8 + 5] = clock64();
+        if (++s == a.stages) { s = 0; ph ^= 1u; }
+        if (TAIL && it > 0) issue_tail(it - 1);
       }
-      if (tr) p.trace[it * 8 + 5] = clock64();
-      if (++s == a.stages) { s = 0; ph ^= 1u; }
       if (TAIL && it > 0) issue_tail(it - 1);
     }
-    if (TAIL && it > 0) issue_tail(it - 1);
   }
 
   tc_fence_before();
@@ -638,7 +785,7 @@
   ConvParams p = p_in;
   a.nsplit = 1;
   static const bool split_env = !getenv("IRMV_NO_NSPLIT");
-  if (split_env && p.w_raster_split && p.split_ways > 1 && p.stride == 1 && !p.in_parity && !p.tail_w && !p.out2 && !p.out_runs &&
+  if (split_env && p.w_raster_split && p.split_ways > 1 && p.stride == 1 && !p.in_parity && !p.tail_w && !p.head_w && !p.out2 && !p.out_runs &&
       !p.seg[0].runs && !p.res_up && p.out && p.cout == p.npad && p.npad % (16 * p.split_ways) == 0) {
     const long long m = (long long)p.B * (p.OH + 1) * (p.OW + 1) - (p.OW + 1);
     if ((m + 127) / 128 * p.split_ways <= num_sms) {
@@ -682,6 +829,17 @@
   const int ext_c = tail ? p.tail_ext.c : 0;
   if (ext_c % 16 || (tail && p.tail_ext.up) || (tail && p.tail_out2 && ((p.OH & 1) || (p.OW & 1)))) return false;
   a.ext_planes = ext_c / 8;
+  const bool head = p.head_w != nullptr;
+  if (head && (tail || p.k != 3 || s2 || p.nseg != 1 || p.seg[0].runs || p.out_runs || p.out2 || p.res_up || !p.act ||
+               p.cin != p.npad || p.cout != p.npad || p.OW + 17 > kGuardFront))
+    return false;
+  const int hcin = head ? p.cin : 0;
+  a.bh_bytes = (uint32_t)((size_t)9 * hcin * hcin * 2);
+  auto head_lead = [&](int R) { return (128 * R - a.Wp - 1) & ~7; };
+  auto head_win_head = [&](int R) { return (128 * R + a.Wp + 1 - head_lead(R) + 7) & ~7; };
+  auto head_bytes = [&](int R) {
+    return head ? (size_t)a.bh_bytes + (size_t)a.NCH * (256 * R + head_win_head(R)) * 16 + 128 + (size_t)hcin * 4 : (size_t)0;
+  };
   a.bt_bytes = tail ? (uint32_t)((size_t)(p.npad + ext_c) * tnp * 2) : 0u;
   int ext_stages = 1;
   auto tail_bytes = [&](int R) { return tail ? (size_t)a.bt_bytes + (size_t)(p.npad + ext_c * ext_stages) * 128 * R * 2 + 256 : (size_t)0; };
@@ -697,18 +855,22 @@
   static const bool ext2_env = !getenv("IRMV_EXT1");
   for (int R = 4; R >= 1 && !best_R; R >>= 1) {
     if (R > rmax_env) continue;
-    if (2 * R * (p.npad + tnp) > 512) continue;
+    if (2 * R * (p.npad + tnp + hcin) > 512) continue;
     long long tiles = (Mr + 128 * R - 1) / (128 * R);
-    if (R > 1 && tiles < 2LL * num_sms) continue;
+    if (head) {
+      if (R < 2 || head_lead(R) < a.Wp + 1 || 256 * R + 8 > a.Wp + kGuardBack) continue;
+    } else if (R > 1 && tiles < 2LL * num_sms) {
+      continue;
+    }
     for (ext_stages = (ext_c && ext2_env) ? 2 : 1; ext_stages >= 1; --ext_stages) {
-      if (a.b_bytes + tail_bytes(R) + 2 * stage_bytes(R) + misc > (size_t)SMEM_BUDGET) continue;
+      if (a.b_bytes + head_bytes(R) + tail_bytes(R) + 2 * stage_bytes(R) + misc > (size_t)SMEM_BUDGET) continue;
       best_R = R;
       break;
     }
   }
   if (ext_stages < 1) ext_stages = 1;
   a.ext_stages = ext_stages;
-  if (!best_R && tail) return false;
+  if (!best_R && (tail || head)) return false;
   if (!best_R && !getenv("IRMV_NO_BSTREAM")) {
     if (p.k == 1) {
       if (a.NCH % 8 != 0 || a.NCH / 8 > 9) return false;
@@ -733,10 +895,14 @@
   a.npix_need = plane_pixels(a.R);
   a.PP = a.npix_need;
   a.a_stage_bytes = (uint32_t)stage_bytes(a.R);
-  int cols = 2 * a.R * (p.npad + tnp), alloc = 32;
+  int cols = 2 * a.R * (p.npad + tnp + hcin), alloc = 32;
   while (alloc < cols) alloc <<= 1;
   a.tmem_cols = alloc;
   a.tmem_tail0 = 2 * a.R * p.npad;
+  a.tmem_head0 = 2 * a.R * (p.npad + tnp);
+  a.lead = head ? head_lead(a.R) : 0;
+  a.win_head = head ? head_win_head(a.R) : 0;
+  a.win_pix = head ? 2 * a.TM + a.win_head : 0;
   a.num_tiles = (int)((Mr + a.TM - 1) / a.TM);
   size_t b_smem = a.b_bytes;
   if (a.b_stream) {
@@ -749,8 +915,8 @@
     b_smem = (size_t)a.b_stages * a.b_tap_bytes;
   } else {
     const size_t half_budget = 112 * 1024;
-    const size_t fixed = a.b_bytes + tail_bytes(a.R) + misc;
-    const bool two = !getenv("IRMV_ONE_CTA") && alloc <= 256 && fixed + 2 * (size_t)a.a_stage_bytes <= half_budget;
+    const size_t fixed = a.b_bytes + head_bytes(a.R) + tail_bytes(a.R) + misc;
+    const bool two = !head && !getenv("IRMV_ONE_CTA") && alloc <= 256 && fixed + 2 * (size_t)a.a_stage_bytes <= half_budget;
     a.ctas_per_sm = two ? 2 : 1;
     const size_t budget = two ? half_budget : (size_t)SMEM_BUDGET;
     a.stages = (int)((budget - fixed) / a.a_stage_bytes);
@@ -764,9 +930,13 @@
   a.off_mid = (uint32_t)((a.off_b + b_smem + 127u) & ~(size_t)127u);
   a.off_ext = a.off_mid + (tail ? (uint32_t)((size_t)p.npad * a.TM * 2) : 0u);
   a.off_bt = a.off_ext + (uint32_t)((size_t)ext_c * a.ext_stages * a.TM * 2);
-  a.off_bias = (uint32_t)((a.off_bt + a.bt_bytes + 127u) & ~(size_t)127u);
+  a.off_bh = a.off_bt + a.bt_bytes;
+  a.off_win = (a.off_bh + a.bh_bytes + 127u) & ~127u;
+  a.off_bias = (uint32_t)((a.off_win + (size_t)a.NCH * a.win_pix * 16 + 127u) & ~(size_t)127u);
   a.off_tbias = a.off_bias + (uint32_t)p.npad * 4;
-  a.off_bars = (a.off_tbias + (uint32_t)tnp * 4 + 15u) & ~15u;
+  a.off_hbias = a.off_tbias + (uint32_t)tnp * 4;
+  a.off_bars = (a.off_hbias + (uint32_t)hcin * 4 + 15u) & ~15u;
+  a.head_idesc = (1u << 4) | ((uint32_t)((head ? hcin : 16) >> 3) << 17) | ((uint32_t)(128 >> 4) << 24);
   a.tail_idesc = (1u << 4) | ((uint32_t)((tail ? tnp : 16) >> 3) << 17) | ((uint32_t)(128 >> 4) << 24);
   for (int t = 0; t < 9; ++t) {
     const int ky = t / 3, kx = t % 3;
@@ -775,6 +945,7 @@
       a.tap_a[t] = (uint32_t)(g * a.NCH * a.PP + delta + (ky == 0 ? 0 : a.Wp) + (kx == 0 ? 0 : 1));
     } else if (a.taps == 9) {
       a.tap_a[t] = (uint32_t)(delta + ky * a.Wp + kx);
+      a.tap_w[t] = head ? (uint32_t)(a.TM - a.lead + (ky - 1) * a.Wp + (kx - 1)) : 0u;
     } else {
       a.tap_a[t] = (uint32_t)(delta + t * 8 * a.PP);
     }
@@ -782,10 +953,10 @@
   return true;
 }
 
-template <int R, int NEPI, bool ACT, int RES, int TAIL>
+template <int R, int NEPI, bool ACT, int RES, int TAIL, bool HEAD = false>
 cudaError_t launch_k(const RArgs &a, int grid, size_t smem, cudaStream_t s) {
   {
-    cudaError_t e = cudaFuncSetAttribute(conv_raster_kernel<R, NEPI, ACT, RES, TAIL>, cudaFuncAttributeMaxDynamicSharedMemorySize, 227 * 1024);
+    cudaError_t e = cudaFuncSetAttribute(conv_raster_kernel<R, NEPI, ACT, RES, TAIL, HEAD>, cudaFuncAttributeMaxDynamicSharedMemorySize, 227 * 1024);
     if (e != cudaSuccess) return e;
   }
   static const bool pdl = !getenv("IRMV_NO_PDL");
@@ -799,12 +970,20 @@
   attr[0].val.programmaticStreamSerializationAllowed = 1;
   cfg.attrs = attr;
   cfg.numAttrs = pdl ? 1 : 0;
-  return cudaLaunchKernelEx(&cfg, conv_raster_kernel<R, NEPI, ACT, RES, TAIL>, a);
+  return cudaLaunchKernelEx(&cfg, conv_raster_kernel<R, NEPI, ACT, RES, TAIL, HEAD>, a);
 }
 
 template <int R, int NEPI>
 cudaError_t launch_r(const RArgs &a, int grid, size_t smem, cudaStream_t s) {
   const bool act = a.p.act != 0, res = a.p.res != nullptr;
+  if (a.p.head_w) {
+    if constexpr (NEPI != 16 || R == 1) {
+      return cudaErrorInvalidValue;
+    } else {
+      if (!act || a.p.tail_w) return cudaErrorInvalidValue;
+      return res ? launch_k<R, NEPI, true, 1, 0, true>(a, grid, smem, s) : launch_k<R, NEPI, true, 0, 0, true>(a, grid, smem, s);
+    }
+  }
   if (res && a.p.res_up) {
     if (!act || a.p.tail_w) return cudaErrorInvalidValue;
     return launch_k<R, NEPI, true, 2, 0>(a, grid, smem, s);
@@ -827,7 +1006,7 @@
   RArgs a;
   if (!p.w_raster || !plan(p, num_sms, a)) return false;
   out[0] = a.R; out[1] = a.ctas_per_sm == 2 ? 8 : 16; out[2] = a.b_stream; out[3] = a.ctas_per_sm; out[4] = a.stages;
-  out[5] = a.b_stages; out[6] = p.tail_w ? (p.tail_act ? 2 : 1) : 0; out[7] = a.num_tiles;
+  out[5] = a.b_stages; out[6] = p.head_w ? 3 : p.tail_w ? (p.tail_act ? 2 : 1) : 0; out[7] = a.num_tiles;
   return true;
 }
 
diff --git a/irmv_detection_b200/csrc/engine.cu b/irmv_detection_b200/csrc/engine.cu
--- a/irmv_detection_b200/csrc/engine.cu
+++ b/irmv_detection_b200/csrc/engine.cu
@@ -330,6 +330,7 @@
   ShuffleUnitParams su{};
   ConvParams cp{};
   bool raster = false;
+  bool c2f_cv1 = false;
   int stream = 0, wait = -1, signal = -1;
   __half *pool_buf = nullptr;
   int pH = 0, pW = 0, pC = 0;
@@ -655,6 +656,7 @@
   if (!split) add_conv(e, ln, cv1, in, H, W, buf, 0);
   for (int i = 0; i < n; ++i) {
     add_conv(e, ln, *e->convs[ci++], {{&buf, (1 + i) * c, c, 0}}, H, W, tmp, 0);
+    ln.ops.back().c2f_cv1 = true;
     add_conv(e, ln, *e->convs[ci++], {{&tmp, 0, c, 0}}, H, W, buf, (2 + i) * c,
              shortcut ? &buf : nullptr, (1 + i) * c);
   }
@@ -706,6 +708,53 @@
     for (auto it = ln.taps.begin(); it != ln.taps.end();)
       it = (it->second.p == o0) ? ln.taps.erase(it) : std::next(it);
     ln.ops.erase(ln.ops.begin() + (long)i + 1);
+  }
+}
+
+void fuse_heads(irmv_engine *e, Lane &ln) {
+  if (e->cfg.conv_impl == IRMV_CONV_DIRECT || e->cfg.reserved[1] || getenv("IRMV_NO_TAIL")) return;
+  auto overlaps = [](const __half *a0, const __half *a1, const __half *b0, const __half *b1) { return a0 < b1 && b0 < a1; };
+  for (size_t i = 0; i + 1 < ln.ops.size(); ++i) {
+    const Op &m = ln.ops[i];
+    Op &b = ln.ops[i + 1];
+    if (m.kind != Op::CONV || b.kind != Op::CONV || !m.raster || !b.raster || !m.c2f_cv1 || m.cp.OH < 80) continue;
+    if ((long long)e->S * (m.cp.OH + 1) * (m.cp.OW + 1) < 2LL * e->num_sms * 512) continue;
+    const ConvParams &mp = m.cp;
+    ConvParams bp = b.cp;
+    if (mp.k != 3 || mp.stride != 1 || mp.nseg != 1 || mp.in_parity || mp.seg[0].runs || mp.seg[0].up || !mp.act) continue;
+    if (mp.res || mp.tail_w || mp.head_w || mp.out2 || mp.out_runs || !mp.out || mp.cout != mp.cin || mp.npad != mp.cout) continue;
+    if (bp.k != 3 || bp.stride != 1 || bp.nseg != 1 || bp.in_parity || bp.head_w || bp.tail_w || bp.H != mp.OH || bp.W != mp.OW) continue;
+    if (bp.seg[0].ptr != mp.out || bp.seg[0].pstride != mp.out_pstride || bp.seg[0].c != mp.cout || bp.seg[0].runs) continue;
+    if (m.stream != b.stream || (m.wait >= 0 && b.wait >= 0) || m.signal >= 0) continue;
+    const __half *o0 = mp.out, *o1 = mp.out + (long long)(mp.cout / 8) * mp.out_pstride;
+    bool other = false;
+    for (size_t j = i + 2; j < ln.ops.size() && !other; ++j) {
+      const Op &q = ln.ops[j];
+      if (q.kind == Op::POOL) { other = overlaps(o0, o1, q.pool_buf, q.pool_buf + 4LL * (q.pC / 8) * q.pStride); continue; }
+      if (q.kind == Op::DW) { other = overlaps(o0, o1, q.dw.in, q.dw.in + (long long)q.dw.planes * q.dw.in_ps); continue; }
+      if (q.kind == Op::SHUF) { other = overlaps(o0, o1, q.su.in, q.su.in + (long long)(q.su.down ? q.su.cin / 8 : q.su.h / 4) * q.su.in_ps); continue; }
+      for (int sgi = 0; sgi < q.cp.nseg; ++sgi) {
+        const ConvSeg &g = q.cp.seg[sgi];
+        if (!q.cp.in_parity && overlaps(o0, o1, g.ptr, g.ptr + (long long)(g.c / 8) * g.pstride)) other = true;
+      }
+      if (q.cp.res && overlaps(o0, o1, q.cp.res, q.cp.res + (long long)(q.cp.cout / 8) * q.cp.res_pstride)) other = true;
+      const ConvSeg &x = q.cp.tail_ext;
+      if (q.cp.tail_w && x.c && overlaps(o0, o1, x.ptr, x.ptr + (long long)(x.c / 8) * x.pstride)) other = true;
+      if (!other && q.cp.out == o0 && q.cp.cout == mp.cout && q.cp.out_pstride == mp.out_pstride) break;
+    }
+    for (int h = 0; h < 3 && !other; ++h)
+      if (ln.heads.box[h] == mp.out || ln.heads.cls[h] == mp.out) other = true;
+    if (other) continue;
+    bp.seg[0] = mp.seg[0];
+    bp.seg[1] = mp.seg[0];
+    bp.head_w = mp.w_raster; bp.head_bias = mp.bias;
+    bp.w_raster_split = nullptr; bp.split_ways = 0;
+    if (!conv_raster_fits(bp)) continue;
+    b.cp = bp;
+    if (m.wait >= 0) b.wait = m.wait;
+    for (auto it = ln.taps.begin(); it != ln.taps.end();)
+      it = (it->second.p == o0) ? ln.taps.erase(it) : std::next(it);
+    ln.ops.erase(ln.ops.begin() + (long)i);
   }
 }
 
@@ -903,6 +952,7 @@
     }
   if (ci != e->convs.size()) { set_error("internal: conv count mismatch"); return false; }
   fuse_tails(e, ln);
+  fuse_heads(e, ln);
   if (!lane_alloc(ln, (void **)&ln.nms.boxes, (size_t)S * kNumAnchors * 16) ||
       !lane_alloc(ln, (void **)&ln.nms.keys, (size_t)S * kNumAnchors * e->nc * 8) ||
       !lane_alloc(ln, (void **)&ln.nms.counts, (size_t)S * 4))
@@ -2085,8 +2135,8 @@
     if (o.kind == Op::POOL) snprintf(line, sizeof line, "pool\n");
     else if (o.kind == Op::DW) snprintf(line, sizeof line, "dw %d %d %d\n", o.dw.stride, o.dw.planes * 8, o.dw.H / o.dw.stride);
     else if (o.kind == Op::SHUF) snprintf(line, sizeof line, "unit %d %d %d %d %d\n", o.su.down, o.su.cin, o.su.h, o.su.H, o.su.TH);
-    else snprintf(line, sizeof line, "conv %d %d %d %d %d %d %d\n", o.cp.k, o.cp.stride, o.cp.cin, o.cp.cout, o.cp.OH,
-                  o.raster ? 1 : 0, o.cp.tail_w ? o.cp.tail_cout : 0);
+    else snprintf(line, sizeof line, "conv %d %d %d %d %d %d %d %d\n", o.cp.k, o.cp.stride, o.cp.cin, o.cp.cout, o.cp.OH,
+                  o.raster ? 1 : 0, o.cp.tail_w ? o.cp.tail_cout : 0, o.cp.head_w ? 1 : 0);
     out += line;
   }
   if ((int)out.size() + 1 > cap) { set_error("buffer too small"); return -1; }
diff --git a/irmv_detection_b200/engine.py b/irmv_detection_b200/engine.py
--- a/irmv_detection_b200/engine.py
+++ b/irmv_detection_b200/engine.py
@@ -228,9 +228,9 @@
             elif f[0] == "unit":
                 ops.append({"kind": "unit", "down": bool(int(f[1])), "cin": int(f[2]), "h": int(f[3]), "hw": int(f[4]), "rows_per_cta": int(f[5])})
             else:
-                k, s, cin, cout, hw, raster, tail = (int(v) for v in f[1:])
+                k, s, cin, cout, hw, raster, tail, head = (int(v) for v in f[1:])
                 ops.append({"kind": "conv", "k": k, "s": s, "cin": cin, "cout": cout, "hw": hw, "raster": bool(raster),
-                            "tail_cout": tail})
+                            "tail_cout": tail, "head": bool(head)})
         return ops
 
     def describe_plans(self, n: int):
```
